# marbl/meryl

Measured on AMD Instinct MI355X. Metric: distinct k-mers counted/sec (whole node), higher is better.
Workload: dtype u64; 1 GPU; meryl count k=21 on synthetic short reads: 66666667 x 150 bp reads per GPU (10.00 Gbp per GPU, 30x of a 333333334 bp genome, 0.5% substitutions, 0.01% N), inputs resident in HBM; k=21, reads_per_gpu=66666667, bases_per_gpu=10066666717, n_distinct=1181289506, parallelism=1 GPU, transport=none (one GPU), n_instances=8648488363, w_prefix=18

## Files before the change

include/meryl_gpu_count.h:

```cpp
#ifndef MERYL_GPU_COUNT_H
#define MERYL_GPU_COUNT_H

#include <stddef.h>
#include <stdint.h>

#ifdef __cplusplus
extern "C" {
#endif

#define MGC_OK            0
#define MGC_EINVAL       -1
#define MGC_ENOMEM       -2
#define MGC_EHIP         -3
#define MGC_ESTATE       -4
#define MGC_EUNSUPPORTED -5
#define MGC_ETIMEOUT     -6
#define MGC_EFORMAT      -7

#define MGC_MODE_CANONICAL 0
#define MGC_MODE_FORWARD   1
#define MGC_MODE_REVERSE   2

#define MGC_NUM_FILES_BITS 6
#define MGC_NUM_FILES      64
// ... 253 lines not shown

int mgc_begin_bam(mgc_session *s);
int mgc_push_bam(mgc_session *s, const void *bam_bytes, size_t len);
int mgc_end_bam(mgc_session *s);
int mgc_push_bam_file(mgc_session *s, const char *path, int threads);
int mgc_dev_bam_decode(const uint8_t *d_piece, uint64_t piece_bytes, const void *d_segments, uint64_t n_segments, uint64_t out_bytes,
                       uint8_t *d_out, void *stream);

int mgc_push_bases_device(mgc_session *s, const uint8_t *d_bases, uint64_t n_bases);

int mgc_staged_bases(mgc_session *s, const uint8_t **d_bases, uint64_t *n_bases);

int mgc_count(mgc_session *s);

int mgc_count_partitioned(mgc_session *s, void *d_keys, const uint64_t *file_counts , void *reserved);

int mgc_count_buckets(mgc_session *s, void *d_keys, uint32_t bucket_bits, const uint64_t *bucket_counts);
int mgc_count_buckets_into(mgc_session *s, void *d_keys, uint32_t bucket_bits, const uint64_t *bucket_counts,
                           void *d_out_keys, uint32_t *d_out_counts, uint64_t capacity, uint64_t *n_distinct,
                           const uint64_t *d_fine_hist );

typedef struct mgc_result_info {
  uint64_t n_bases;
  uint64_t n_instances;
  uint64_t n_distinct;
  uint32_t w_prefix, w_data;
  uint64_t n_prefix;
  uint64_t file_instances[MGC_NUM_FILES];
} mgc_result_info;
int mgc_get_result_info(const mgc_session *s, mgc_result_info *info);

int mgc_copy_result_device(mgc_session *s, void *d_keys_out, uint32_t *d_counts_out);

int mgc_get_result_device(const mgc_session *s, const void **d_unique, const uint32_t **d_counts,
                          const uint64_t **d_block_start, uint32_t *key_words);

int mgc_copy_result(const mgc_session *s, uint64_t *keys_lo, uint64_t *keys_hi, uint32_t *counts,
                    uint64_t *block_start);

typedef int (*mgc_block_cb)(void *ctx, uint64_t prefix, uint64_t n_kmers,
                            const uint64_t *suffix_lo, const uint64_t *suffix_hi,
                            const uint32_t *counts);
int mgc_finish(mgc_session *s, mgc_block_cb cb, void *ctx, int host_threads);

typedef int (*mgc_block_cb2)(void *ctx, uint64_t prefix, uint64_t n_kmers,
                             const uint64_t *suffix_lo, const uint64_t *suffix_hi,
                             const uint32_t *counts, const uint64_t *labels, uint64_t label);
int mgc_finish_labelled(mgc_session *s, mgc_block_cb2 cb, void *ctx, int host_threads);

#define MGC_STAGE_HISTOGRAM 0
#define MGC_STAGE_PARTITION 1
#define MGC_STAGE_SORT      2
#define MGC_STAGE_RLE       3
#define MGC_STAGE_BLOCKS    4
#define MGC_NUM_STAGES      5
typedef struct mgc_profile {
  double   stage_ms[MGC_NUM_STAGES];
  uint32_t stage_launches[MGC_NUM_STAGES];
  double   sort_pass_ms_total;
  uint32_t sort_pass_launches;
  uint64_t sort_pass_keys;
  double   total_ms;
  double   merge_ms;
  uint32_t n_batches;
  uint32_t narrow_digit_widths;
  double   pass_ms[2];
  uint64_t pass_bytes[2];
  uint64_t pass_keys[2];
  uint32_t pass_launches[2];
  double   finish_ms;
  uint64_t finish_bytes, finish_keys;
  uint32_t finish_launches;
  uint32_t wide_msd_files;
  uint32_t stream_files;
  uint32_t k96_files;
  uint32_t k96_widened_files;
  uint32_t hpc_mixed_files;
  uint64_t stream_retries;
  double   probe_ratio;
  double   pack_ms;
  uint64_t hist_bytes;
  uint64_t partition_bytes;
  uint32_t pass_kernel_launches[2];
} mgc_profile;
int mgc_set_profiling(mgc_session *s, int enable);
int mgc_get_profile(const mgc_session *s, mgc_profile *p);

int mgc_dev_synth_reads(uint64_t seed, uint64_t genome_len, uint64_t first_read, uint64_t n_reads,
                        uint32_t read_len, uint32_t sub_rate_ppm, uint32_t n_rate_ppm,
                        uint8_t *d_out, void *stream);
int mgc_dev_synth_reads_ex(uint64_t seed, uint64_t genome_len, uint64_t first_read, uint64_t n_reads,
                           uint32_t read_len, uint32_t sub_rate_ppm, uint32_t n_rate_ppm,
                           uint32_t repeat_ppm, uint32_t repeat_unit, uint32_t repeat_families,
                           uint8_t *d_out, void *stream);

uint32_t mgc_version(void);

#ifdef __cplusplus
}
#endif
#endif
```

meryl_amd/build.py:

```python
import os
import shutil
import subprocess
import sys

HERE = os.path.dirname(os.path.abspath(__file__))
CSRC = os.path.join(HERE, "csrc")
LIB = os.path.join(HERE, "libmeryl_gpu_count.so")
SOURCES = ["mgc_kmer.hip", "mgc_sort.hip", "mgc_scan.hip", "mgc_finish.hip", "mgc_misc.hip", "mgc_parse.hip",
           "mgc_encode.hip", "mgc_decode.hip", "mgc_merge.hip", "mgc_merge_many.hip", "mgc_lookup.hip", "mgc_filter.hip", "mgc_import.hip", "mgc_analyze.hip", "mgc_value_hist.hip", "mgc_positions.hip", "mgc_list.hip", "mgc_bam.hip", "mgc_gzip.hip",
           "mgc_api.cpp", "mgc_textfile.cpp", "mgc_import.cpp", "mgc_analyze.cpp", "mgc_dbfile.cpp", "mgc_positions.cpp", "mgc_count.cpp", "mgc_stream.cpp", "mgc_eval.cpp", "mgc_runs.cpp", "mgc_node.cpp", "meryl_db.cpp", "meryl_seq.cpp"]
HEADERS = ["mgc_device.h", "mgc_common.hpp", "mgc_compact.hpp", "mgc_bases.hpp", "mgc_stream_geom.hpp", "mdb_layout.h", "mdb_statistics.hpp", "mgc_session.hpp", "mgc_devbuf.hpp", "mgc_dbfile.hpp", "mgc_hist_list.hpp", "mgc_clock.hpp", "mgc_chunk_ring.hpp", "mgc_bgzf.hpp", "mgc_bam_walk.hpp", "mgc_gzip_par.hpp", "mgc_runs.hpp", "mgc_lookup_dev.hpp", "mgc_import_dev.hpp", "mgc_analyze_dev.hpp", "mgc_positions_dev.hpp", "mgc_fastx.hpp", "mgc_label.hpp", "mgc_selector.hpp", "mgc_value.hpp", "mgc_route.hpp", "mgc_group_route.hpp", "mgc_group_batch.hpp", "mgc_list.hpp",
           os.path.join("..", "..", "include", "meryl_gpu_count.h"),
           os.path.join("..", "..", "include", "meryl_db.h"), os.path.join("..", "..", "include", "meryl_seq.h"),
           os.path.join("..", "..", "include", "meryl_lookup.h"), os.path.join("..", "..", "include", "meryl_import.h"),
           os.path.join("..", "..", "include", "meryl_import_labelled.h"),
           os.path.join("..", "..", "include", "meryl_analyze.h"), os.path.join("..", "..", "include", "meryl_positions.h"),
           os.path.join("..", "..", "include", "meryl_list.h")]
OBJDIR = os.path.join(HERE, "build")
CFLAGS = ["--offload-arch=gfx950", "-O3", "-std=c++17", "-fPIC", "-pthread", "-Wall", "-Wno-unused-function"]
LFLAGS = ["--offload-arch=gfx950", "-shared", "-fPIC", "-pthread", "-no-hip-rt"]


def hipcc():
    for cand in (os.environ.get("HIPCC"), shutil.which("hipcc"), "/opt/rocm/bin/hipcc"):
        if cand and os.path.exists(cand):
            return cand
    raise RuntimeError("hipcc not found: the native library cannot be built")


def _sources():
    return [f for f in SOURCES if os.path.exists(os.path.join(CSRC, f))]


def _header_mtime():
    deps = [os.path.join(CSRC, f) for f in HEADERS if os.path.exists(os.path.join(CSRC, f))]
    deps.append(os.path.abspath(__file__))
    return max(os.path.getmtime(d) for d in deps)


def _obj(f):
    return os.path.join(OBJDIR, f + ".o")


def _stale_objects(force=False):
    ht = _header_mtime()
    out = []
    for f in _sources():
        o = _obj(f)
        if force or not os.path.exists(o) or os.path.getmtime(o) < max(os.path.getmtime(os.path.join(CSRC, f)), ht):
            out.append(f)
    return out


def _stale():
    if not os.path.exists(LIB):
        return True
    t = os.path.getmtime(LIB)
    if max([_header_mtime()] + [os.path.getmtime(os.path.join(CSRC, f)) for f in _sources()]) <= t:
        return False
    if _stale_objects():
        return True
    return any(os.path.getmtime(_obj(f)) > t for f in _sources())


CLI = os.path.join(HERE, "bin", "meryl")
LOOKUP_CLI = os.path.join(HERE, "bin", "meryl-lookup")
IMPORT_CLI = os.path.join(HERE, "bin", "meryl-import")
ANALYZE_CLI = os.path.join(HERE, "bin", "meryl-analyze")
POSITION_LOOKUP_CLI = os.path.join(HERE, "bin", "position-lookup")


def _build_front_end(source, out, force, verbose, headers=()):
    src = os.path.join(CSRC, source)
    newest = max(os.path.getmtime(os.path.join(CSRC, f)) for f in (source,) + tuple(headers))
    if (not force and os.path.exists(out) and os.path.getmtime(out) >= newest
            and os.path.getmtime(out) >= os.path.getmtime(LIB)):
        return out
    os.makedirs(os.path.dirname(out), exist_ok=True)
    rocm_lib = os.path.join(os.environ.get("ROCM_PATH", "/opt/rocm"), "lib")
    tmp = "%s.tmp%d" % (out, os.getpid())
    cmd = [hipcc(), "-O2", "-std=c++17", "-pthread", src, "-o", tmp, "-L" + HERE, "-lmeryl_gpu_count",
           "-Wl,-rpath,$ORIGIN/..", "-L" + rocm_lib, "-lamdhip64", "-Wl,-rpath," + rocm_lib, "-lz"]
    if verbose:
        print(" ".join(cmd), file=sys.stderr)
    subprocess.check_call(cmd)
    os.replace(tmp, out)
    return out


def build_cli(force=False, verbose=False):
    return _build_front_end("meryl_main.cpp", CLI, force, verbose)


def build_lookup_cli(force=False, verbose=False):
# ... 57 lines not shown
```

meryl_amd/capi.py:

```python
import ctypes
import os

from . import build as _build

MGC_OK, MGC_EINVAL, MGC_ENOMEM, MGC_EHIP, MGC_ESTATE, MGC_EUNSUPPORTED, MGC_ETIMEOUT = 0, -1, -2, -3, -4, -5, -6
MODE_CANONICAL, MODE_FORWARD, MODE_REVERSE = 0, 1, 2
NUM_FILES = 64
NUM_STAGES = 5
STAGE_NAMES = ("histogram", "partition", "sort", "rle", "blocks")

SYMBOLS = (
    "mgc_configure_counting", "mgc_format_configured_line",
    "mgc_dev_partition_workspace_bytes", "mgc_dev_kmer_histogram", "mgc_dev_kmer_partition",
    "mgc_dev_sort_workspace_bytes", "mgc_dev_radix_sort", "mgc_dev_radix_group", "mgc_dev_kmer_histogram_fine",
    "mgc_dev_rle_workspace_bytes", "mgc_dev_rle_count", "mgc_dev_rle_emit", "mgc_dev_block_offsets",
    "mgc_open", "mgc_close", "mgc_last_error", "mgc_push_bases", "mgc_push_bases_device", "mgc_staged_bases", "mgc_reserve_text", "mgc_begin_text", "mgc_push_text", "mgc_end_text", "mgc_push_text_file", "mgc_push_text_file_range", "mgc_text_record_start", "mgc_push_text_bgzf_file", "mgc_is_bgzf_file", "mgc_begin_bam", "mgc_push_bam", "mgc_end_bam", "mgc_push_bam_file", "mgc_dev_bam_decode", "mgc_push_text_gzip_file", "mgc_is_gzip_file", "mgc_dev_gzip_resolve", "mgc_dev_crc32_pieces", "mgc_count", "mgc_count_partitioned", "mgc_count_buckets", "mgc_count_buckets_into", "mgc_copy_result_device",
    "mgc_get_result_info", "mgc_get_result_device", "mgc_copy_result", "mgc_finish", "mgc_finish_labelled",
    "mgc_set_profiling", "mgc_get_profile", "mgc_dev_synth_reads", "mgc_dev_synth_reads_ex", "mgc_version",
    "mgc_dev_merge_workspace_bytes", "mgc_dev_merge_count", "mgc_dev_merge_count_values", "mgc_dev_merge_emit",
    "mgc_dev_merge_many_tile", "mgc_dev_merge_many_workspace_bytes", "mgc_dev_merge_many_count", "mgc_dev_merge_many_emit",
    "mgc_dev_select_workspace_bytes", "mgc_dev_select_count", "mgc_dev_select_emit",
    "mgc_label_default_constant", "mgc_dev_merge_many_emit_labelled", "mgc_dev_select_emit_labelled", "mgc_dev_decode_blocks", "mgc_dev_buffers_live",
    "mgc_select_parse", "mgc_select_check", "mgc_dev_merge_many_count_selected", "mgc_dev_merge_many_emit_selected",
    "mgc_dev_select_count_selected", "mgc_dev_select_emit_selected",
# ... 78 lines not shown
        ("base_mask", ctypes.c_uint8),
        ("reserved", ctypes.c_uint8 * 3),
        ("lhs_index", ctypes.c_int32),
        ("rhs_index", ctypes.c_int32),
        ("lhs_constant", ctypes.c_uint64),
        ("rhs_constant", ctypes.c_uint64),
        ("count_mask", ctypes.c_uint64),
        ("required_mask", ctypes.c_uint32),
        ("reserved2", ctypes.c_uint32),
    ]


class EvalNodeSelected(ctypes.Structure):
    _fields_ = EvalNodeLabelled._fields_ + [
        ("first_term", ctypes.c_uint32),
        ("n_terms", ctypes.c_uint32),
    ]


class EvalNodeAssigned(ctypes.Structure):
    _fields_ = EvalNodeSelected._fields_ + [
        ("value_assign", ctypes.c_int32),
        ("reserved2", ctypes.c_int32),
        ("value_constant", ctypes.c_uint64),
    ]


ASSIGN_OPS = {"none": 0, "set": 1, "first": 2, "selected": 3, "min": 4, "max": 5, "add": 6, "sum": 6, "sub": 7, "dif": 7, "mul": 8, "div": 9,
              "divzero": 10, "mod": 11, "rem": 11, "count": 12}
SEL_VALUE, SEL_LABEL, SEL_BASES, SEL_INPUT = 1, 2, 3, 4
REL_EQ, REL_NEQ, REL_LEQ, REL_GEQ, REL_LT, REL_GT = 1, 2, 3, 4, 5, 6
SELECT_MAX_TERMS = 16
NODE_DATABASE, NODE_MERGE, NODE_VALUE = 0, 1, 2
LABEL_OPS = {"default": 0, "set": 1, "first": 2, "min": 3, "max": 4, "and": 5, "or": 6, "xor": 7, "difference": 8, "lightest": 9,
             "heaviest": 10, "invert": 11, "selected": 12}
EVAL_SLICE_LABELLED_CB = ctypes.CFUNCTYPE(None, ctypes.c_void_p, ctypes.c_uint32, ctypes.POINTER(ctypes.c_uint64), ctypes.POINTER(ctypes.c_uint64),
                                          ctypes.POINTER(ctypes.c_uint32), ctypes.POINTER(ctypes.c_uint64), ctypes.c_uint64)
EVAL_SLICE_CB = ctypes.CFUNCTYPE(None, ctypes.c_void_p, ctypes.c_uint32, ctypes.POINTER(ctypes.c_uint64), ctypes.POINTER(ctypes.c_uint64),
                                 ctypes.POINTER(ctypes.c_uint32), ctypes.c_uint64)


class ResultInfo(ctypes.Structure):
    _fields_ = [
        ("n_bases", ctypes.c_uint64),
        ("n_instances", ctypes.c_uint64),
        ("n_distinct", ctypes.c_uint64),
        ("w_prefix", ctypes.c_uint32),
        ("w_data", ctypes.c_uint32),
        ("n_prefix", ctypes.c_uint64),
        ("file_instances", ctypes.c_uint64 * NUM_FILES),
    ]


class Profile(ctypes.Structure):
    _fields_ = [
        ("stage_ms", ctypes.c_double * NUM_STAGES),
        ("stage_launches", ctypes.c_uint32 * NUM_STAGES),
        ("sort_pass_ms_total", ctypes.c_double),
        ("sort_pass_launches", ctypes.c_uint32),
        ("sort_pass_keys", ctypes.c_uint64),
        ("total_ms", ctypes.c_double),
        ("merge_ms", ctypes.c_double),
        ("n_batches", ctypes.c_uint32),
        ("narrow_digit_widths", ctypes.c_uint32),
        ("pass_ms", ctypes.c_double * 2),
        ("pass_bytes", ctypes.c_uint64 * 2),
        ("pass_keys", ctypes.c_uint64 * 2),
        ("pass_launches", ctypes.c_uint32 * 2),
        ("finish_ms", ctypes.c_double),
        ("finish_bytes", ctypes.c_uint64),
        ("finish_keys", ctypes.c_uint64),
        ("finish_launches", ctypes.c_uint32),
        ("wide_msd_files", ctypes.c_uint32),
        ("stream_files", ctypes.c_uint32),
        ("k96_files", ctypes.c_uint32),
        ("k96_widened_files", ctypes.c_uint32),
        ("hpc_mixed_files", ctypes.c_uint32),
        ("stream_retries", ctypes.c_uint64),
        ("probe_ratio", ctypes.c_double),
        ("pack_ms", ctypes.c_double),
        ("hist_bytes", ctypes.c_uint64),
        ("partition_bytes", ctypes.c_uint64),
        ("pass_kernel_launches", ctypes.c_uint32 * 2),
    ]


class DbInfo(ctypes.Structure):
    _fields_ = [
        ("k", ctypes.c_uint32),
        ("prefix_size", ctypes.c_uint32),
        ("suffix_size", ctypes.c_uint32),
        ("num_files_bits", ctypes.c_uint32),
        ("num_blocks_bits", ctypes.c_uint32),
        ("flags", ctypes.c_uint32),
        ("num_unique", ctypes.c_uint64),
        ("num_distinct", ctypes.c_uint64),
        ("num_total", ctypes.c_uint64),
        ("hist_len", ctypes.c_uint64),
        ("label_size", ctypes.c_uint32),
        ("reserved", ctypes.c_uint32),
    ]


class NodeProfile(ctypes.Structure):
    _fields_ = [
        ("n_ranks", ctypes.c_uint32),
        ("bucket_bits", ctypes.c_uint32),
        ("n_bases", ctypes.c_uint64),
        ("n_instances", ctypes.c_uint64),
        ("n_distinct", ctypes.c_uint64),
        ("data_bytes", ctypes.c_uint64),
        ("partition_s", ctypes.c_double),
        ("exchange_count_s", ctypes.c_double),
        ("close_s", ctypes.c_double),
        ("merge_parts_s", ctypes.c_double),
        ("total_s", ctypes.c_double),
        ("n_batches", ctypes.c_uint32),
        ("n_host_runs", ctypes.c_uint32),
        ("host_run_bytes", ctypes.c_uint64),
        ("merge_runs_s", ctypes.c_double),
        ("peak_hbm_bytes", ctypes.c_uint64),
    ]

    def as_dict(self):
        return {n: getattr(self, n) for n, _ in self._fields_}


class DbWriteProfile(ctypes.Structure):
    _fields_ = [
        ("plan_ms", ctypes.c_double),
        ("encode_ms", ctypes.c_double),
        ("copy_write_s", ctypes.c_double),
        ("total_s", ctypes.c_double),
        ("data_bytes", ctypes.c_uint64),
        ("n_kmers", ctypes.c_uint64),
        ("n_blocks", ctypes.c_uint64),
    ]

    def as_dict(self):
        return {n: getattr(self, n) for n, _ in self._fields_}


class RunsProfile(ctypes.Structure):
    _fields_ = [
        ("n_runs", ctypes.c_uint32), ("n_host_runs", ctypes.c_uint32),
        ("n_entries", ctypes.c_uint64),
        ("device_bytes", ctypes.c_uint64), ("host_bytes", ctypes.c_uint64),
        ("n_merged", ctypes.c_uint64),
        ("n_chunks", ctypes.c_uint32),
        ("spill_s", ctypes.c_double),
        ("upload_s", ctypes.c_double), ("merge_ms", ctypes.c_double), ("deliver_s", ctypes.c_double),
        ("peak_hbm_bytes", ctypes.c_uint64),
    ]

    def as_dict(self):
        return {n: getattr(self, n) for n, _ in self._fields_}


class GzipInfo(ctypes.Structure):
    _fields_ = [(n, ctypes.c_uint64) for n in ("members", "chunks", "confirmed", "discarded", "text_bytes", "symbol_bytes", "cuts")]


class LookupInfo(ctypes.Structure):
    _fields_ = [("k", ctypes.c_uint32), ("key_words", ctypes.c_uint32), ("index_bits", ctypes.c_uint32), ("reserved", ctypes.c_uint32),
                ("n_kmers", ctypes.c_uint64), ("n_kmers_in_db", ctypes.c_uint64), ("device_bytes", ctypes.c_uint64)]

# ... 381 lines not shown
```

meryl_amd/csrc/mgc_api.cpp:

```cpp
#include "../../include/meryl_gpu_count.h"
#include "mgc_device.h"
#include "mgc_session.hpp"
#include "mgc_gzip_par.hpp"
#include "mgc_runs.hpp"
#include "mgc_selector.hpp"
#include "mgc_value.hpp"

#include <algorithm>
#include <cstdio>
#include <cstdlib>
#include <cstring>
#include <string>
#include <thread>
#include <vector>

namespace mgc {
std::string &thread_last_error() {
  thread_local std::string e;
  return e;
}

Switches read_switches() {
  Switches sw;
  auto off = [](const char *n) { const char *e = getenv(n); return e && e[0] == '0'; };
  auto on1 = [](const char *n) { const char *e = getenv(n); return e && e[0] == '1'; };
  auto num = [](const char *n, uint64_t d) { const char *e = getenv(n); return (e && *e) ? strtoull(e, nullptr, 10) : d; };
  sw.fine_hist = !off("MGC_FINE_HIST"); sw.hpc_msd = !off("MGC_HPC_MSD"); sw.hpc_digits = !off("MGC_HPC_DIGITS");
  sw.const_k = !off("MGC_KMER_CONST_K"); sw.packed_bases = !off("MGC_PACKED_BASES"); sw.narrow = !off("MGC_NARROW"); sw.wide_msd = !off("MGC_WIDE_MSD");
  sw.group_pipe = !off("MGC_GROUP_PIPE"); sw.soa5 = !off("MGC_SOA5"); sw.k96 = !off("MGC_K96"); sw.finish = !off("MGC_FINISH");
  sw.nolist = on1("MGC_FINISH_NOLIST");
  sw.finish_trace = getenv("MGC_FINISH_TRACE") != nullptr; sw.group_dbg = getenv("MGC_GROUP_DBG") != nullptr; sw.hash_dbg = getenv("MGC_HASH_DBG") != nullptr;
  { const char *e = getenv("MGC_HASH_MULTI"); sw.hash_multi = (e && *e) ? atoi(e) : -1; }
  { const char *e = getenv("MGC_HASH_STREAM"); sw.hash_stream = (e && *e) ? atoi(e) : -1; }
  sw.min_top = (uint32_t)num("MGC_FINISH_MIN_TOP", 0);
  sw.finish_target = num("MGC_FINISH_TARGET", 0);
  sw.stream_max = num("MGC_STREAM_MAX", (uint64_t)1 << 22);
  sw.bucket_bases = num("MGC_BUCKET_BASES", 0);
  sw.huge_streams = (uint32_t)num("MGC_HUGE_STREAMS", 4);
  sw.huge_slices = !off("MGC_HUGE_SLICES");
  sw.pass_stagger = (uint32_t)num("MGC_PASS_STAGGER", 0);
  sw.group_batch_bytes = num("MGC_GROUP_BATCH_BYTES", sw.group_batch_bytes);
  sw.group_batch_files = (uint32_t)num("MGC_GROUP_BATCH_FILES", 0);
  return sw;
}
}
using mgc::set_err;

namespace {


uint64_t number_of_bits64(uint64_t v) {
  uint64_t b = 0;
  while (v) { b++; v >>= 1; }
  return b;
}

uint64_t expected_simple_size(uint32_t k, uint64_t n_est, uint32_t suffix_len) {
  if (2 * k - 2 * suffix_len > 42) return UINT64_MAX;
  const uint64_t low_bits  = 16;
  const uint64_t n_entries = (uint64_t)1 << (2 * k - 2 * suffix_len);
  const uint64_t exp_max   = (uint64_t)(0.004 * (double)n_est);
  const uint64_t exp_bits  = number_of_bits64(exp_max) + 1;
  const uint64_t extra     = (exp_bits < low_bits) ? 0 : (exp_bits - low_bits);
  return (n_entries * low_bits + n_entries * extra) / 8;
}

void best_prefix_size(const mgc_count_config &c, uint64_t n_est, uint64_t mem_allowed, uint32_t *best,
                      uint64_t *mem_used) {
  const uint32_t k = c.k;
  const uint32_t seg_bits = c.page_size * 8, seg_bytes = c.page_size;
  *best = 0;
  *mem_used = UINT64_MAX;
  for (uint32_t wp = 1; wp < 2 * k - 1; wp++) {
    const uint64_t n_prefix = (uint64_t)1 << wp;
    const uint64_t kpp = n_est / n_prefix + 1;
    const uint64_t kps = seg_bits / (2 * k - wp);
    const uint64_t spp = kpp / kps + 1;
    if (wp + number_of_bits64(spp) + number_of_bits64(seg_bytes) >= 64) break;
    const uint64_t struct_mem = (uint64_t)c.sizeof_count_array * n_prefix + 8 * n_prefix * spp;
    const uint64_t data_min   = n_prefix * seg_bytes;
    const uint64_t total      = struct_mem + n_prefix * spp * seg_bytes;
    if (struct_mem + data_min > mem_allowed) break;
    if ((wp > 9) && (total + (uint64_t)16 * wp * 1024 * 1024 < *mem_used)) {
      *mem_used = total;
      *best = wp;
    }
    if (total > (uint64_t)16 * *mem_used) break;
  }
}

}

extern "C" uint32_t mgc_version(void) { return (0u << 16) | 3u; }

extern "C" int mgc_configure_counting(mgc_count_config *c) {
  if (!c) return MGC_EINVAL;
  if (c->k == 0 || c->k > 64) {
    set_err(nullptr, "ERROR: Kmer size not supplied with modifier k=<kmer-size>.");
    return MGC_EINVAL;
  }
  if (c->mode < 0 || c->mode > 2) return MGC_EINVAL;
  if (c->page_size == 0) c->page_size = 4096;
  if (c->sizeof_count_array == 0) c->sizeof_count_array = 3232;

  c->use_simple = 0; c->w_prefix = 0; c->n_prefix = 0; c->w_data = 0; c->n_batches = 1; c->memory_used = 0;

  const uint64_t mem_simple = expected_simple_size(c->k, c->n_kmers_estimate, c->count_suffix_length);
  uint64_t mem_complex = UINT64_MAX;
  uint32_t best = 0, n_batches = 1;

  if (c->k > 5) {
    for (n_batches = 1; mem_complex > c->memory_allowed; n_batches++) {
      best_prefix_size(*c, c->n_kmers_estimate / n_batches, c->memory_allowed, &best, &mem_complex);
      if (n_batches > (1u << 20)) {
        set_err(nullptr, "configureCounting: no prefix size fits in %lu bytes", (unsigned long)c->memory_allowed);
        return MGC_EINVAL;
      }
    }
    c->w_prefix = best;
    c->n_prefix = (uint64_t)1 << best;
    c->w_data   = 2 * c->k - best;
  }
  if ((mem_simple < mem_complex) && (mem_simple < c->memory_allowed)) {
    c->use_simple = 1; c->memory_used = mem_simple;
  } else {
// ... 469 lines not shown
    if (2 * cfg->k - 2 * sfx_len > 42) {
      set_err(nullptr, "mgc_open: count-suffix forces simple mode, which takes at most 21 free bases (k - suffix length = %u)", cfg->k - sfx_len);
      return nullptr;
    }
    for (uint32_t i = 0; i < sfx_len; i++) {
      const char ch = cfg->count_suffix[i];
      const bool ok = ch == 'A' || ch == 'C' || ch == 'G' || ch == 'T' || ch == 'a' || ch == 'c' || ch == 'g' || ch == 't';
      if (!ok) { set_err(nullptr, "mgc_open: count-suffix '%s' holds something that is not ACGT", cfg->count_suffix); return nullptr; }
      sfx_test = (sfx_test << 2) | (uint64_t)(((unsigned char)ch >> 1) & 3);
    }
    sfx_mask = (sfx_len == 32) ? ~0ull : (((uint64_t)1 << (2 * sfx_len)) - 1);
    eff.use_simple = 1;
  }
  if (!mgc::effective_geometry(&eff)) return nullptr;
  cfg = &eff;
  if (cfg->k == 0 || cfg->k > 64 || cfg->w_prefix < MGC_NUM_FILES_BITS || cfg->w_prefix > 2 * cfg->k ||
      cfg->w_data != 2 * cfg->k - cfg->w_prefix) {
    set_err(nullptr, "mgc_open: config has not been through mgc_configure_counting (k=%u wPrefix=%u wData=%u)",
            cfg->k, cfg->w_prefix, cfg->w_data);
    return nullptr;
  }

  int ndev = 0;
  hipError_t e = hipGetDeviceCount(&ndev);
  if (e != hipSuccess || ndev == 0) {
    set_err(nullptr, "mgc_open: no HIP device (%s)", hipGetErrorString(e));
    return nullptr;
  }
  mgc_session *s = new mgc_session();
  s->cfg = *cfg;
  s->sfx_mask = sfx_mask;
  s->sfx_test = sfx_test;
  s->key_words = (cfg->k > 32) ? 2u : 1u;
  if (device >= 0) {
    e = hipSetDevice(device);
    if (e != hipSuccess) { set_err(nullptr, "hipSetDevice(%d): %s", device, hipGetErrorString(e)); delete s; return nullptr; }
    s->device = device;
  } else {
    (void)hipGetDevice(&s->device);
  }
  e = hipStreamCreateWithFlags(&s->stream, hipStreamNonBlocking);
  if (e == hipSuccess) e = hipStreamCreateWithFlags(&s->st_in, hipStreamNonBlocking);
  if (e != hipSuccess) { set_err(nullptr, "hipStreamCreate: %s", hipGetErrorString(e)); delete s; return nullptr; }
  if (hipStreamCreateWithFlags(&s->stream2, hipStreamNonBlocking) != hipSuccess ||
      hipEventCreateWithFlags(&s->ev_fork, hipEventDisableTiming) != hipSuccess ||
      hipEventCreateWithFlags(&s->ev_join, hipEventDisableTiming) != hipSuccess) {
    set_err(nullptr, "hipStreamCreate / hipEventCreate failed"); mgc_close(s); return nullptr;
  }
  memset(&s->prof, 0, sizeof(s->prof));
  memset(s->file_instances, 0, sizeof(s->file_instances));
  memset(s->total_file_instances, 0, sizeof(s->total_file_instances));
  s->sw = mgc::read_switches();
  return s;
}

extern "C" void mgc_close(mgc_session *s) {
  if (!s) return;
  if (s->worker_active) { s->worker.join(); s->worker_active = false; }
  s->join_prepare();
  (void)hipSetDevice(s->device);
  if (s->st_in) (void)hipStreamSynchronize(s->st_in);
  s->free_result();
  s->free_garbage();
  s->free_arena();
  delete s->runs;
  s->runs = nullptr;
  for (int i = 0; i < 2; i++) {
    if (s->text_pinned[i]) (void)hipHostFree(s->text_pinned[i]);
    if (s->text_ev[i]) (void)hipEventDestroy(s->text_ev[i]);
    if (s->up_ev[i]) (void)hipEventDestroy(s->up_ev[i]);
    if (s->pin[i]) (void)hipHostFree(s->pin[i]);
    if (s->pin_ev[i]) (void)hipEventDestroy(s->pin_ev[i]);
    if (s->bam_seg_pinned[i]) (void)hipHostFree(s->bam_seg_pinned[i]);
    if (s->gz_sym_pinned[i]) (void)hipHostFree(s->gz_sym_pinned[i]);
    if (s->gz_tab_pinned[i]) (void)hipHostFree(s->gz_tab_pinned[i]);
  }
  for (char *&p : s->text_ring) if (p) { (void)hipHostFree(p); p = nullptr; }
  if (s->st_up) { (void)hipStreamSynchronize(s->st_up); (void)hipStreamDestroy(s->st_up); }
  if (s->st_in) (void)hipStreamDestroy(s->st_in);
  if (s->ev_fork) (void)hipEventDestroy(s->ev_fork);
  if (s->h_stats) (void)hipHostFree(s->h_stats);
  if (s->ev_join) (void)hipEventDestroy(s->ev_join);
  if (s->stream2) (void)hipStreamDestroy(s->stream2);
  for (int i = 0; i < mgc_session::HUGE_EXTRA; i++) if (s->stream_h[i]) (void)hipStreamDestroy(s->stream_h[i]);
  if (s->stream) (void)hipStreamDestroy(s->stream);
  delete s;
}

struct HostParseState { uint64_t out_len, file_start_len; uint32_t state, prev_nl, error, pad; };

static int count_staged_batch(mgc_session *s, int which, uint64_t n);

extern "C" int mgc_prepare(mgc_session *s, uint64_t expected_bases) {
  if (!s) return MGC_EINVAL;
  if (s->borrowed || s->counted || s->prep_active || expected_bases == 0) return MGC_OK;
  HIP_TRY(s, hipSetDevice(s->device));
  size_t free_b = 0, total_b = 0;
  if (hipMemGetInfo(&free_b, &total_b) != hipSuccess) return MGC_OK;
  const uint64_t per_base = 2 + 14ull * s->key_words;
  if (s->batch_limit && expected_bases > s->batch_limit) return MGC_OK;
  if ((double)expected_bases * (double)per_base > 0.8 * (double)free_b) return MGC_OK;
  const size_t bytes = sizeof(uint64_t) * s->key_words * expected_bases;
  s->prep_active = true;
  s->prep_thread = std::thread([s, bytes] {
    (void)hipSetDevice(s->device);
    if (s->ensure(mgc_session::B_X, bytes) != hipSuccess) (void)hipGetLastError();
    (void)mgc::warm_kmer(); (void)mgc::warm_scan(); (void)mgc::warm_sort(); (void)mgc::warm_finish(); (void)mgc::warm_encode(); (void)mgc::warm_value_hist();
    (void)hipGetLastError();
  });
  return MGC_OK;
}

extern "C" int mgc_set_batch_bases(mgc_session *s, uint64_t bases_per_batch) {
  if (!s) return MGC_EINVAL;
  s->batch_limit = bases_per_batch;
  return MGC_OK;
}

static inline int stage_id(int which) { return which ? mgc_session::B_STAGE1 : mgc_session::B_STAGE0; }
static inline uint8_t *stage_ptr(mgc_session *s, int which) { return reinterpret_cast<uint8_t *>(s->buf[stage_id(which)].p); }

static int input_setup(mgc_session *s) {
  if (s->borrowed || s->counted) { set_err(&s->err, "input after device input / count"); return MGC_ESTATE; }
  HIP_TRY(s, hipSetDevice(s->device));
  if (s->state_ready) return MGC_OK;
  if (s->batch_limit == 0) {
    size_t free_b = 0, total_b = 0;
    if (hipMemGetInfo(&free_b, &total_b) == hipSuccess && free_b) {
      const uint64_t per_base = 2 + 14ull * s->key_words;
      s->batch_limit = (uint64_t)((double)free_b * 0.80 / (double)per_base);
    }
    if (s->batch_limit < (1u << 20)) s->batch_limit = 1u << 20;
  }
  HIP_TRY(s, s->ensure(mgc_session::B_TEXT_STATE, mgc::text_parse_state_bytes() + 64));
  HIP_TRY(s, s->ensure_preserve(stage_id(s->fill), 1u << 20, 0, s->st_in));
  HIP_TRY(s, mgc::launch_text_file_op(s->buf[mgc_session::B_TEXT_STATE].p, stage_ptr(s, s->fill), 3, s->st_in));
  s->state_ready = true;
  return MGC_OK;
}

static int resolve_length(mgc_session *s, HostParseState *out = nullptr) {
  HostParseState h;
  HIP_TRY(s, hipMemcpyAsync(&h, s->buf[mgc_session::B_TEXT_STATE].p, sizeof(h), hipMemcpyDeviceToHost, s->st_in));
  HIP_TRY(s, hipStreamSynchronize(s->st_in));
  s->fill_len = h.out_len;
  s->len_inexact = false;
  if (out) *out = h;
  return MGC_OK;
}

static int join_worker(mgc_session *s) {
  if (s->worker_active) {
    const double t0 = mgc::now_s();
    s->worker.join();
    s->tr_join += mgc::now_s() - t0;
    s->worker_active = false;
    if (s->worker_rc != MGC_OK) return s->worker_rc;
  }
  return s->worker_rc;
}

static int flush_pinned(mgc_session *s) {
  if (s->pin_len == 0) return MGC_OK;
  if (s->len_inexact) { const int rc = resolve_length(s); if (rc != MGC_OK) return rc; }
  const int c = s->pin_cur;
  HIP_TRY(s, s->ensure_preserve(stage_id(s->fill), s->fill_len + s->pin_len + 4096, s->fill_len, s->st_in));
// ... 767 lines not shown
```

meryl_amd/csrc/mgc_count.cpp:

```cpp
#include "mgc_session.hpp"
#include "mgc_group_batch.hpp"
#include "mgc_group_route.hpp"

#include <algorithm>
#include <vector>

#define TRY(expr) do { const int rc__ = (expr); if (rc__ != MGC_OK) return rc__; } while (0)

namespace {
using S = mgc_session;

struct StageTimer {
  bool on;
  hipStream_t st;
  hipEvent_t ev[MGC_NUM_STAGES][2];
  bool used[MGC_NUM_STAGES];
  StageTimer(bool enable, hipStream_t s) : on(enable), st(s) {
    for (int i = 0; i < MGC_NUM_STAGES; i++) {
      used[i] = false;
      if (on) { (void)hipEventCreate(&ev[i][0]); (void)hipEventCreate(&ev[i][1]); }
    }
  }
  ~StageTimer() {
    if (on) for (int i = 0; i < MGC_NUM_STAGES; i++) { (void)hipEventDestroy(ev[i][0]); (void)hipEventDestroy(ev[i][1]); }
  }
  void begin(int i) { if (on) { (void)hipEventRecord(ev[i][0], st); used[i] = true; } }
  void end(int i)   { if (on) (void)hipEventRecord(ev[i][1], st); }
};

enum class Group : uint8_t {
  NONE,
  SORT,
  NARROW,
  WIDE,
};

struct FilePlan {
  uint64_t size = 0, start = 0;
  uint32_t top = 0;
  uint32_t top_str = 0;
  mgc::SortPlan sp{};
  Group kind = Group::NONE;
  bool hpc = false;
  bool hpc_stream = false;
  bool hpc_cand = false;
  bool hpc_mixed = false;
  bool stream = false;
  bool k96 = false;
  bool msd_ok = true;
  uint32_t tr_a = 0, tr_b = 0;
  uint64_t gbase = 0, sbase = 0, slots = 0;
  size_t nws_off = 0;
  uint32_t *cnt = nullptr;
  uint64_t maxsub = 0, nlarge = 0, nzcount = 0;
  bool fallback = false;
  uint32_t passes = 0; bool narrowed = false, k96_passes = false;
  int batch_lead = -1;
  uint64_t ngf() const { return size ? (uint64_t)1 << top : 0; }
};

uint32_t plan_bucket_bits(const mgc_count_config &c, const mgc::Switches &sw, uint64_t n_bases) {
  const uint64_t per_bucket = sw.bucket_bases ? sw.bucket_bases
                                              : (c.homopoly_compress ? 60000000ull : 180000000ull);
  const uint32_t step = c.homopoly_compress ? 2u : 1u;
  uint32_t bits = MGC_NUM_FILES_BITS;
  while (bits + step <= MGC_MAX_BUCKET_BITS && bits + step <= 2 * c.k && (n_bases >> bits) > per_bucket) bits += step;
  return bits;
}

struct CountPlan {
  const mgc_count_config &c;
  const mgc::Switches &sw;
  mgc_profile &prof;
  uint32_t kw, bucket_bits, nb, rem_bits, fine_bits;
  bool fine = false;
  bool fine_hpc = false;
  uint64_t max_bucket = 0, ng_total = 0, ns_total = 0;
  uint64_t target = 0, cap = 0, starget = 0;
  bool stream_on = false, hpc_ok = false, hpc_stream_ok = false, hpc_mixed_ok = false;
  std::vector<FilePlan> files;

  CountPlan(const mgc_count_config &c_, const mgc::Switches &sw_, mgc_profile &prof_, uint32_t kw_, uint32_t bucket_bits_)
      : c(c_), sw(sw_), prof(prof_), kw(kw_), bucket_bits(bucket_bits_), nb(1u << bucket_bits_), rem_bits(2 * c_.k - bucket_bits_),
        fine_bits(15u - bucket_bits_), files(nb) {}

// ... 120 lines not shown
    }
  }

  int choose_probe() {
    bool any_cand = false;
    for (const FilePlan &x : files) any_cand = any_cand || x.top_str != 0 || x.hpc_cand;
    if (!any_cand) return -1;
    if (sw.hash_stream == 1) {
      for (FilePlan &x : files) if (x.top_str) take_coarser(x);
      return -1;
    }
    int probe = -1;
    uint64_t best = ~0ull;
    for (uint32_t b = 0; b < nb; b++)
      if (files[b].size >= max_bucket / 16 && files[b].size >= 4096 && files[b].size < best) { best = files[b].size; probe = (int)b; }
    return probe;
  }
  void apply_probe(uint32_t probe) {
    for (uint32_t b = 0; b < nb; b++)
      if (b != probe && (files[b].top_str || (files[b].hpc_cand && !files[b].stream))) take_coarser(files[b]);
  }

  uint32_t soa_mask(bool plain_input) const {
    bool soa = sw.soa5 && plain_input && kw == 1 && nb == 64 && fine && rem_bits > 32 && rem_bits <= 40;
    for (const FilePlan &x : files) if (x.size && !(x.kind == Group::NARROW && x.top)) soa = false;
    return soa ? (1u << (rem_bits - 32)) - 1u : 0u;
  }
  bool k96_layout(bool plain_input) {
    if (!(sw.k96 && plain_input && kw == 2 && nb == 64 && fine && rem_bits <= 96 && !c.homopoly_compress)) return false;
    bool any = false;
    for (FilePlan &x : files) if (x.size && x.kind == Group::WIDE && x.top) { x.k96 = true; any = true; prof.k96_files++; }
    return any;
  }
};

struct Count {
  mgc_session *s;
  const mgc::CountInput &in;
  hipStream_t st;
  const mgc_count_config &c;
  const mgc::Switches &sw;
  mgc_profile &prof;
  const uint32_t k, kw, bucket_bits, nb, rem_bits;
  const size_t kbytes;
  CountPlan plan;
  StageTimer tm;
  hipEvent_t ev_all[2] = {nullptr, nullptr};

  const uint8_t *d_bases;
  uint64_t n_bases, N = 0, nd = 0;
  void *part_ws = nullptr, *sort_ws = nullptr, *rle_ws = nullptr;
  uint64_t *d_counts64 = nullptr, *d_starts = nullptr;
  std::vector<uint64_t> h_meta;
  const uint64_t *d_fine = nullptr, *d_fine_hpc = nullptr;
  void *d_packed = nullptr;
  mgc::SortPlan full{};
  bool use_finish;
  unsigned char *X = nullptr, *Y = nullptr;
  size_t sort_ws_bytes = 0;
  uint32_t *d_err = nullptr;
  uint32_t soa_hi_mask = 0;
  static constexpr uint32_t ev_per_file = 2 * 16;
  std::vector<hipEvent_t> pass_ev;
  uint32_t sort_launch_groups = 0;
  size_t y_base_bytes = 0;
  std::vector<unsigned char> h_batch_tables;
  int group_dbg_left = 2;

  int probe = -1;
  uint64_t *d_substart = nullptr, *d_group = nullptr, *d_stats = nullptr, *d_retrycnt = nullptr;
  uint32_t *d_large = nullptr, *d_nz = nullptr;
  const size_t hdr_bytes = mgc::sort_header_bytes();
  unsigned char *d_nws = nullptr, *d_nhdrs = nullptr;
  std::vector<mgc::DBuf> cnt_extra;
  bool fork_huge = false, forked = false, need_join = false;
  static constexpr int NH = 1 + S::HUGE_EXTRA;
  hipStream_t hstream[NH] = {};
  unsigned char *halt[NH] = {};
  void *hws[NH] = {nullptr, nullptr, nullptr, nullptr};
  size_t hws_bytes = 0;
  int n_huge_streams = 1, huge_next = 0;
  std::vector<std::pair<hipEvent_t, hipEvent_t>> fin_ev;
  uint64_t fin_keys = 0, fin_in_bytes = 0; bool fin_narrow = false;

  Count(mgc_session *s_, const mgc::CountInput &in_, uint32_t bucket_bits_)
      : s(s_), in(in_), st(s_->stream), c(s_->cfg), sw(s_->sw), prof(s_->prof), k(c.k), kw(s_->key_words), bucket_bits(bucket_bits_),
        nb(1u << bucket_bits_), rem_bits(2 * c.k - bucket_bits_), kbytes(sizeof(uint64_t) * kw), plan(c, sw, s_->prof, kw, bucket_bits_),
        tm(s_->profiling, s_->stream), d_bases(s_->d_bases), n_bases(s_->n_bases), h_meta(2 * (size_t)nb, 0), use_finish(sw.finish) {}

  void *seg(uint32_t b) const { return X + kbytes * plan.files[b].start; }
  uint32_t low(const FilePlan &x) const { return rem_bits - x.top; }
  const uint32_t *nz_list(const FilePlan &x) const { return (4 * x.nzcount < 3 * x.ngf() && !sw.nolist) ? d_nz + x.gbase : nullptr; }
  bool msd_file(const FilePlan &x) const {
    return d_fine_hpc ? x.kind == Group::WIDE : (x.kind == Group::NARROW || x.kind == Group::WIDE) && x.msd_ok;
  }
  mgc::FinishFile finish_desc(uint32_t b, bool stream, hipStream_t fst, int hsel) const;
  void take_stats(uint32_t b) {
    const uint64_t *h = s->h_stats + 3 * (size_t)b;
    plan.files[b].maxsub = h[0]; plan.files[b].nlarge = h[1]; plan.files[b].nzcount = h[2];
  }

  int run();
  int compress_bases(); int histogram(); int buffers(); int partition(bool soa, bool k96);
  int count_full();
  int count_finish(); int finish_buffers(); int prepare_headers(); int narrow_prepare(int only, int skip);
  int probe_file(); int group_file(uint32_t b); int stats_file(uint32_t b); int group_all();
  mgc::GroupFile group_desc(uint32_t b); bool batch_file(uint32_t b) const; int group_batches();
  int huge_setup(); int huge_sync_all(); int huge_join_all();
  int finish_file(uint32_t b); int oversized_streams(uint32_t b, bool *stream); int widen_back(uint32_t b, bool *unordered);
  int count_file(uint32_t b, bool stream); int fallback_file(uint32_t b, bool unordered);
  int trace_slices(); int retry(); int scan_pack(); int pack_file(uint32_t b); void finish_profile();
  int block_offsets(); void collect_profile();
};

int Count::compress_bases() {
  if (!c.homopoly_compress || !n_bases || in.keys) return MGC_OK;
  HIP_TRY(s, s->ensure(S::B_HPC, n_bases));
  HIP_TRY(s, s->ensure(S::B_HPC_WS, mgc::hpc_workspace_bytes(n_bases)));
  uint8_t *d_hpc = reinterpret_cast<uint8_t *>(s->buf[S::B_HPC].p);
  void *hws_ = s->buf[S::B_HPC_WS].p;
  HIP_TRY(s, mgc::launch_homopoly_compress(d_bases, n_bases, d_hpc, hws_, st));
  uint64_t n_out = 0;
  HIP_TRY(s, hipMemcpyAsync(&n_out, hws_, sizeof(uint64_t), hipMemcpyDeviceToHost, st));
  HIP_TRY(s, hipStreamSynchronize(st));
  d_bases = d_hpc;
  n_bases = n_out;
  return MGC_OK;
}

int Count::histogram() {
  HIP_TRY(s, s->ensure(S::B_PART_WS, mgc::kp_workspace_bytes(bucket_bits)));
  HIP_TRY(s, s->ensure(S::B_META, sizeof(uint64_t) * nb * 3));
  part_ws = s->buf[S::B_PART_WS].p;
  d_counts64 = reinterpret_cast<uint64_t *>(s->buf[S::B_META].p);
  d_starts = d_counts64 + nb;
  std::vector<uint64_t> h_counts(nb);
  const bool wide_msd_on = sw.wide_msd && !c.homopoly_compress;
  if (!in.keys) {
    if (sw.packed_bases && n_bases) {
      const size_t pb = mgc::kp_packed_bytes(n_bases);
      bool room = s->buf[S::B_PACKED].cap >= pb;
      if (!room) {
        size_t free_b = 0, total_b = 0;
        room = hipMemGetInfo(&free_b, &total_b) == hipSuccess &&
               (double)free_b + (double)s->arena_bytes() >= (double)n_bases * (double)(2 + 14ull * kw) + (double)pb;
      }
      if (room) {
        if (s->ensure(S::B_PACKED, pb) == hipSuccess) d_packed = s->buf[S::B_PACKED].p;
        else (void)hipGetLastError();
      }
    }
    tm.begin(MGC_STAGE_HISTOGRAM);
    if (n_bases >= (1u << 22) && ((kw == 1 && 2 * k - bucket_bits <= 41) || wide_msd_on) && mgc::kmer_histogram_fine_ok(k, bucket_bits, s->sfx_mask, sw)) {
      HIP_TRY(s, s->ensure(S::B_FINE, sizeof(uint64_t) << 15));
      uint64_t *fine = reinterpret_cast<uint64_t *>(s->buf[S::B_FINE].p);
      HIP_TRY(s, mgc::launch_kmer_histogram_fine(d_bases, n_bases, k, c.mode, d_counts64, fine, part_ws, st, sw.const_k, 6, d_packed));
      d_fine = fine;
    } else if (c.homopoly_compress && n_bases >= (1u << 22) && (2 * k - bucket_bits) % 2 == 0 && 2 * k - bucket_bits >= 20 &&
               sw.hpc_digits && mgc::kmer_histogram_hpc_ok(k, bucket_bits, s->sfx_mask, sw)) {
      HIP_TRY(s, s->ensure(S::B_FINE, sizeof(uint64_t) * std::max<size_t>((size_t)1 << 15, mgc::kmer_histogram_hpc_entries(bucket_bits))));
      uint64_t *fine = reinterpret_cast<uint64_t *>(s->buf[S::B_FINE].p);
      HIP_TRY(s, mgc::launch_kmer_histogram_hpc(d_bases, n_bases, k, c.mode, bucket_bits, d_counts64, fine, part_ws, st, sw.const_k, d_packed));
      d_fine_hpc = fine;
    } else
    HIP_TRY(s, mgc::launch_kmer_histogram(d_bases, n_bases, k, c.mode, bucket_bits, d_counts64, part_ws, st, s->sfx_mask, s->sfx_test, d_packed));
    tm.end(MGC_STAGE_HISTOGRAM);
    prof.stage_launches[MGC_STAGE_HISTOGRAM] = 1;
    HIP_TRY(s, hipMemcpyAsync(h_counts.data(), d_counts64, sizeof(uint64_t) * nb, hipMemcpyDeviceToHost, st));
    HIP_TRY(s, hipStreamSynchronize(st));
  } else {
    memcpy(h_counts.data(), in.counts, sizeof(uint64_t) * nb);
    uint64_t n_ext = 0;
    for (uint32_t b = 0; b < nb; b++) n_ext += h_counts[b];
    if (in.fine && sw.fine_hist && bucket_bits <= 8 && n_ext >= (1u << 22) && s->sfx_mask == 0 && !c.homopoly_compress &&
        2 * k >= 15 + 2 && ((kw == 1 && 2 * k - bucket_bits <= 41) || wide_msd_on))
      d_fine = in.fine;
  }
  memset(s->file_instances, 0, sizeof(s->file_instances));
  for (uint32_t b = 0; b < nb; b++) {
    plan.files[b].size = h_counts[b];
    plan.files[b].start = h_meta[b] = N;
    N += h_counts[b];
    plan.max_bucket = std::max(plan.max_bucket, h_counts[b]);
    s->file_instances[b >> (bucket_bits - MGC_NUM_FILES_BITS)] += h_counts[b];
  }
  s->n_instances = N;
  plan.fine = d_fine != nullptr;
  plan.fine_hpc = d_fine_hpc != nullptr;
  return MGC_OK;
}

int Count::buffers() {
  mgc::make_sort_plan(0, rem_bits, &full);
  const bool odd = !use_finish && (full.num_passes & 1u) != 0;
// ... 348 lines not shown
  if (*stream && x.maxsub > sw.stream_max && kw == 2) {
    *stream = false;
  } else if (*stream && x.maxsub > sw.stream_max) {
    uint32_t h_fail[3] = {0, 0, 0};
    HIP_TRY(s, hipMemsetAsync(d_err + 4, 0, 12, st));
    HIP_TRY(s, mgc::launch_finish_probe(finish_desc(b, true, st, 0), sw.stream_max, d_err + 4));
    HIP_TRY(s, hipMemcpyAsync(h_fail, d_err + 4, 12, hipMemcpyDeviceToHost, st));
    HIP_TRY(s, hipStreamSynchronize(st));
    *stream = (h_fail[0] == 0);
    if (sw.finish_trace)
      fprintf(stderr, "[finish] bucket %u: largest sub-bucket %llu > %llu, up to %u distinct in one: %s\n", b,
              (unsigned long long)x.maxsub, (unsigned long long)sw.stream_max, h_fail[2],
              *stream ? "streamed through the hash tables" : "too many distinct: stable-sort fallback");
  } else if (sw.finish_trace && x.maxsub > plan.cap) {
    fprintf(stderr, "[finish] bucket %u: largest sub-bucket %llu > %llu: %s\n", b, (unsigned long long)x.maxsub,
            (unsigned long long)plan.cap, *stream ? "streamed through the hash tables" : "stable-sort fallback");
  }
  return MGC_OK;
}

int Count::widen_back(uint32_t b, bool *unordered) {
  FilePlan &x = plan.files[b];
  if (need_join) TRY(huge_sync_all());
  forked = false;
  if (x.k96) {
    const unsigned __int128 fb = (unsigned __int128)b << rem_bits;
    HIP_TRY(s, mgc::launch_widen_k96(seg(b), x.size, (uint64_t)fb, (uint64_t)(fb >> 64), (void *)Y, st));
  } else {
    HIP_TRY(s, mgc::launch_widen_groups(seg(b), d_substart + x.sbase, x.ngf(), (uint64_t)b << rem_bits, low(x), (void *)Y, st, x.tr_a, x.tr_b));
  }
  HIP_TRY(s, hipMemcpyAsync(seg(b), Y, kbytes * x.size, hipMemcpyDeviceToDevice, st));
  if (x.k96) {
    x.k96 = false;
    prof.k96_widened_files++;
    return MGC_OK;
  }
  x.kind = Group::SORT;
  *unordered = x.tr_a != 0;
  if (x.stream) { x.stream = false; *unordered = true; }
  cnt_extra.emplace_back();
  HIP_TRY(s, cnt_extra.back().ensure(sizeof(uint32_t) * x.size));
  x.cnt = reinterpret_cast<uint32_t *>(cnt_extra.back().p);
  return MGC_OK;
}

mgc::FinishFile Count::finish_desc(uint32_t b, bool stream, hipStream_t fst, int hsel) const {
  const FilePlan &x = plan.files[b];
  mgc::FinishFile f;
  f.keys = seg(b); f.alt = halt[hsel];
  f.layout = x.kind == Group::NARROW ? mgc::FinishKeys::NARROW32 : x.k96 ? mgc::FinishKeys::K96 : kw == 2 ? mgc::FinishKeys::WHOLE16 : mgc::FinishKeys::WHOLE8;
  f.starts = d_substart + x.sbase; f.ng = x.ngf(); f.low_bits = low(x); f.tr_a = x.tr_a; f.tr_b = x.tr_b;
  f.n_keys = x.size; f.max_sub = x.maxsub;
  f.cnt_tmp = x.cnt; f.group_distinct = d_group + x.gbase;
  f.large_list = d_large + x.gbase; f.n_large = x.nlarge; f.stream = stream;
  f.nonempty_list = nz_list(x); f.nonempty_count = d_stats + 3 * (size_t)b + 2;
  f.retry_list = x.stream ? d_large + x.gbase + x.nlarge : d_nz + x.gbase; f.retry_count = d_retrycnt + b;
  f.stream_cap = x.stream ? mgc::finish_stream_capacity() : 0;
  f.huge_ws = hws[hsel]; f.huge_ws_bytes = hws_bytes; f.huge_ws_keys = plan.max_bucket; f.d_error = d_err;
  f.st = fst; f.st_huge = hstream[hsel];
  f.hash_multi = sw.hash_multi; f.hash_dbg = sw.hash_dbg;
  return f;
}

int Count::count_file(uint32_t b, bool stream) {
  const FilePlan &x = plan.files[b];
  const bool on_second = fork_huge && (b & 1u);
  if ((stream || on_second) && fork_huge && !forked) {
    HIP_TRY(s, hipEventRecord(s->ev_fork, st));
    for (int i = 0; i < n_huge_streams; i++) HIP_TRY(s, hipStreamWaitEvent(hstream[i], s->ev_fork, 0));
    forked = need_join = true;
  }
  hipStream_t fst = on_second ? s->stream2 : st;
  const int hsel = (stream && x.nlarge > 0 && n_huge_streams > 1) ? (huge_next++ % n_huge_streams) : 0;
  const bool narrow = x.kind == Group::NARROW;
  if (s->profiling) {
    fin_ev.emplace_back(); (void)hipEventCreate(&fin_ev.back().first); (void)hipEventCreate(&fin_ev.back().second);
    (void)hipEventRecord(fin_ev.back().first, fst);
    fin_keys += x.size;
    fin_in_bytes += x.size * (narrow ? 4u : (x.k96 ? 12u : (uint64_t)kbytes));
    fin_narrow = fin_narrow || narrow;
  }
  HIP_TRY(s, mgc::launch_finish_file(finish_desc(b, stream, fst, hsel)));
  if (s->profiling) (void)hipEventRecord(fin_ev.back().second, fst);
  return MGC_OK;
}

int Count::fallback_file(uint32_t b, bool unordered) {
  FilePlan &x = plan.files[b];
  x.fallback = true;
  if (need_join) TRY(huge_sync_all());
  forked = false;
  if (low(x) || unordered) {
    int in_alt = 0;
    HIP_TRY(s, mgc::launch_radix_sort(seg(b), (void *)Y, x.size, kw, full, sort_ws, sort_ws_bytes - 256, d_err, &in_alt, st, nullptr));
    if (in_alt) HIP_TRY(s, hipMemcpyAsync(seg(b), Y, kbytes * x.size, hipMemcpyDeviceToDevice, st));
  }
  uint64_t distinct = 0;
  HIP_TRY(s, mgc::launch_rle_count(seg(b), x.size, kw, rle_ws, st));
  HIP_TRY(s, mgc::rle_read_total(rle_ws, &distinct, st));
  HIP_TRY(s, hipMemsetAsync(d_group + x.gbase, 0, sizeof(uint64_t) * x.slots, st));
  HIP_TRY(s, hipMemcpyAsync(d_group + x.gbase, &distinct, sizeof(uint64_t), hipMemcpyHostToDevice, st));
  HIP_TRY(s, hipStreamSynchronize(st));
  return MGC_OK;
}

int Count::trace_slices() {
  if (!sw.finish_trace || !hws[0]) return MGC_OK;
  HIP_TRY(s, hipStreamSynchronize(st));
  for (int i = 0; i < n_huge_streams; i++) {
    if (!hws[i]) continue;
    mgc::HugeTrace t;
    HIP_TRY(s, mgc::finish_huge_trace(hws[i], plan.max_bucket, &t));
    fprintf(stderr, "[finish] sliced count, stream %d: the last file had %u sub-buckets cut into %u slices; %u of them dense (counted by ranges)\n", i, t.cut, t.slices, t.dense);
  }
  return MGC_OK;
}

int Count::retry() {
  bool any_stream = false;
  for (const FilePlan &x : plan.files) any_stream = any_stream || (x.stream && !x.fallback && x.size);
  if (!any_stream) return MGC_OK;
  std::vector<uint64_t> h_retry(nb, 0);
  HIP_TRY(s, hipMemcpyAsync(h_retry.data(), d_retrycnt, sizeof(uint64_t) * nb, hipMemcpyDeviceToHost, st));
  HIP_TRY(s, hipStreamSynchronize(st));
  for (uint32_t b = 0; b < nb; b++) {
    const FilePlan &x = plan.files[b];
    if (!x.stream || x.fallback || h_retry[b] == 0) continue;
    prof.stream_retries += h_retry[b];
    HIP_TRY(s, mgc::launch_finish_retry(finish_desc(b, true, st, 0), h_retry[b]));
  }
  return MGC_OK;
}

int Count::scan_pack() {
  hipEvent_t ev_pack[2] = {nullptr, nullptr};
  if (s->profiling) { (void)hipEventCreate(&ev_pack[0]); (void)hipEventCreate(&ev_pack[1]); (void)hipEventRecord(ev_pack[0], st); }
  HIP_TRY(s, mgc::launch_finish_scan(d_group, plan.ng_total, s->buf[S::B_GSCAN].p, st));
  HIP_TRY(s, hipMemcpyAsync(&nd, d_group + plan.ng_total, sizeof(uint64_t), hipMemcpyDeviceToHost, st));
  HIP_TRY(s, hipStreamSynchronize(st));
  if (plan.ng_total == 0) nd = 0;
  s->n_distinct = nd;
  if (in.out_keys && in.out_counts && nd <= in.out_cap) {
    s->d_unique = in.out_keys;
    s->d_counts = in.out_counts;
  } else {
    HIP_TRY(s, s->ensure(S::B_UNIQUE, kbytes * nd));
    HIP_TRY(s, s->ensure(S::B_COUNTS, sizeof(uint32_t) * nd));
    s->d_unique = s->buf[S::B_UNIQUE].p;
    s->d_counts = reinterpret_cast<uint32_t *>(s->buf[S::B_COUNTS].p);
  }
  for (uint32_t b = 0; b < nb; b++) TRY(pack_file(b));
  if (s->profiling) (void)hipEventRecord(ev_pack[1], st);
  tm.end(MGC_STAGE_RLE);
  prof.stage_launches[MGC_STAGE_RLE] = 4 * nb;
  if (s->profiling) {
    HIP_TRY(s, hipStreamSynchronize(st));
    { float pms = 0; if (hipEventElapsedTime(&pms, ev_pack[0], ev_pack[1]) == hipSuccess) prof.pack_ms = pms; }
    (void)hipEventDestroy(ev_pack[0]); (void)hipEventDestroy(ev_pack[1]);
    finish_profile();
  }
  return MGC_OK;
}

int Count::pack_file(uint32_t b) {
  const FilePlan &x = plan.files[b];
  if (x.size == 0) return MGC_OK;
  void *sg = seg(b);
  if (x.kind == Group::NARROW) {
    HIP_TRY(s, mgc::launch_compact_groups_narrow(sg, x.cnt, d_substart + x.sbase, d_group + x.gbase, x.ngf(), (uint64_t)b << rem_bits, low(x),
                                                 s->d_unique, s->d_counts, st, x.tr_a, x.tr_b, nz_list(x), x.nzcount));
  } else if (!x.fallback && x.k96) {
    const unsigned __int128 fb = (unsigned __int128)b << rem_bits;
    HIP_TRY(s, mgc::launch_compact_groups_k96(sg, x.cnt, d_substart + x.sbase, d_group + x.gbase, x.ngf(), (uint64_t)fb, (uint64_t)(fb >> 64),
                                              s->d_unique, s->d_counts, st, x.tr_a, x.tr_b, nz_list(x), x.nzcount));
  } else if (!x.fallback) {
    HIP_TRY(s, mgc::launch_compact_groups(sg, kw, x.cnt, d_substart + x.sbase, d_group + x.gbase, x.ngf(), s->d_unique, s->d_counts, st,
                                          x.tr_a, x.tr_b, nz_list(x), x.nzcount));
  } else {
    HIP_TRY(s, mgc::launch_rle_count(sg, x.size, kw, rle_ws, st));
    HIP_TRY(s, mgc::launch_rle_emit(sg, x.size, kw, rle_ws, s->d_unique, s->d_counts, st, d_group + x.gbase));
  }
  return MGC_OK;
}

void Count::finish_profile() {
  for (auto &pe : fin_ev) {
    float ms = 0;
    if (hipEventElapsedTime(&ms, pe.first, pe.second) == hipSuccess) { prof.finish_ms += ms; prof.finish_launches++; }
    (void)hipEventDestroy(pe.first); (void)hipEventDestroy(pe.second);
  }
  prof.finish_keys = fin_keys;
  prof.finish_bytes = fin_in_bytes + nd * (fin_narrow ? 8u : (uint64_t)kbytes + 4u);
}

int Count::count_finish() {
  plan.plan_files();
  probe = plan.choose_probe();
  TRY(finish_buffers());
  soa_hi_mask = plan.soa_mask(!in.keys && s->sfx_mask == 0);
  const bool k96 = plan.k96_layout(!in.keys && s->sfx_mask == 0);
  for (uint32_t b = 0; b < nb; b++) h_meta[nb + b] = plan.files[b].k96 ? 1 : 0;
  TRY(partition(soa_hi_mask != 0, k96));
  uint64_t wide_total = 0;
  for (const FilePlan &x : plan.files) if (x.kind != Group::NARROW) wide_total += x.size;
  HIP_TRY(s, s->ensure(S::B_CNT_TMP, sizeof(uint32_t) * wide_total));
  uint32_t *wide = reinterpret_cast<uint32_t *>(s->buf[S::B_CNT_TMP].p);
  uint64_t at = 0;
  for (uint32_t b = 0; b < nb; b++) {
    FilePlan &x = plan.files[b];
    if (x.kind == Group::NARROW) x.cnt = reinterpret_cast<uint32_t *>(seg(b)) + x.size;
    else { x.cnt = wide + at; at += x.size; }
  }
  tm.begin(MGC_STAGE_SORT);
  TRY(prepare_headers());
  if (s->h_stats_cap < 3 * (size_t)nb) {
    if (s->h_stats) { (void)hipHostFree(s->h_stats); s->h_stats = nullptr; s->h_stats_cap = 0; }
    HIP_TRY(s, hipHostMalloc(reinterpret_cast<void **>(&s->h_stats), sizeof(uint64_t) * 3 * (size_t)nb, hipHostMallocDefault));
    s->h_stats_cap = 3 * (size_t)nb;
  }
  fork_huge = s->stream2 != nullptr;
  hstream[0] = fork_huge ? s->stream2 : st;
  halt[0] = Y;
  hws_bytes = mgc::finish_huge_workspace_bytes(plan.max_bucket);
  if (probe >= 0) TRY(probe_file());
  TRY(group_all());
  for (uint32_t b = 0; b < nb; b++) if ((int)b != probe) TRY(finish_file(b));
  if (need_join) TRY(huge_join_all());
  TRY(trace_slices());
  TRY(retry());
  return scan_pack();
}

int Count::block_offsets() {
  HIP_TRY(s, s->ensure(S::B_BLOCKS, sizeof(uint64_t) * (c.n_prefix + 1)));
  s->d_block_start = reinterpret_cast<uint64_t *>(s->buf[S::B_BLOCKS].p);
  tm.begin(MGC_STAGE_BLOCKS);
  HIP_TRY(s, mgc::launch_block_offsets(s->d_unique, nd, kw, c.w_data, c.n_prefix, s->d_block_start, st));
  tm.end(MGC_STAGE_BLOCKS);
  prof.stage_launches[MGC_STAGE_BLOCKS] = 1;
  uint32_t h_err[3] = {0, 0, 0};
  HIP_TRY(s, hipMemcpyAsync(h_err, d_err, sizeof(h_err), hipMemcpyDeviceToHost, st));
  if (s->profiling) (void)hipEventRecord(ev_all[1], st);
  HIP_TRY(s, hipStreamSynchronize(st));
  if (h_err[0]) { mgc::set_err(&s->err, "radix sort look-back timed out"); return MGC_ETIMEOUT; }
  if (h_err[2]) { mgc::set_err(&s->err, "count stage: the retry table of the distinct-sized count filled up, a sub-bucket was not counted"); return MGC_EHIP; }
  return MGC_OK;
}

void Count::collect_profile() {
  float ms = 0;
  for (int i = 0; i < MGC_NUM_STAGES; i++)
    if (tm.used[i] && hipEventElapsedTime(&ms, tm.ev[i][0], tm.ev[i][1]) == hipSuccess) prof.stage_ms[i] = ms;
  if (hipEventElapsedTime(&ms, ev_all[0], ev_all[1]) == hipSuccess) prof.total_ms = ms;
  prof.stage_launches[MGC_STAGE_SORT] = sort_launch_groups * (full.num_passes + 2);
  for (uint32_t b = 0; b < nb; b++) {
    const FilePlan &x = plan.files[b];
    if (x.size == 0) continue;
    const bool follower = x.batch_lead >= 0 && (uint32_t)x.batch_lead != b;
    for (uint32_t p = 0; p < x.passes; p++) {
      hipEvent_t *pe = &pass_ev[(size_t)b * ev_per_file + 2 * p];
      ms = 0;
      if (!follower && hipEventElapsedTime(&ms, pe[0], pe[1]) != hipSuccess) continue;
      if (!follower) prof.pass_kernel_launches[p ? 1 : 0]++;
      prof.sort_pass_ms_total += ms;
      prof.sort_pass_launches++;
      prof.sort_pass_keys += x.size;
      const int pi = p ? 1 : 0;
      prof.pass_ms[pi] += ms;
      prof.pass_launches[pi]++;
      prof.pass_keys[pi] += x.size;
      if (x.narrowed && !p) prof.narrow_digit_widths |= 1u << (x.tr_a ? x.tr_a : x.sp.pass_bits[0]);
      prof.pass_bytes[pi] += x.size * (x.narrowed ? (p ? 8u : (soa_hi_mask ? 9u : 12u)) : (x.k96_passes ? 24u : 2u * kbytes));
    }
  }
  for (auto &e : pass_ev) (void)hipEventDestroy(e);
  (void)hipEventDestroy(ev_all[0]); (void)hipEventDestroy(ev_all[1]);
  (void)hipGetLastError();
}

int Count::run() {
  TRY(compress_bases());
  if (s->profiling) { (void)hipEventCreate(&ev_all[0]); (void)hipEventCreate(&ev_all[1]); (void)hipEventRecord(ev_all[0], st); }
  TRY(histogram());
  TRY(buffers());
  TRY(use_finish ? count_finish() : count_full());
  TRY(block_offsets());
  if (s->profiling) collect_profile();
  return MGC_OK;
}
}

int mgc::count_device(mgc_session *s, const CountInput &in) {
  s->join_prepare();
  s->free_result();
  HIP_TRY(s, hipSetDevice(s->device));
  const uint32_t bucket_bits = in.keys ? in.bucket_bits : plan_bucket_bits(s->cfg, s->sw, s->n_bases);
  memset(&s->prof, 0, sizeof(s->prof));
  Count count(s, in, bucket_bits);
  return count.run();
}
```

meryl_amd/csrc/mgc_device.h:

```cpp
#pragma once

#include <hip/hip_runtime.h>
#include <stddef.h>
#include <stdint.h>
#include "mgc_label.hpp"
#include "../../include/meryl_gpu_count.h"

namespace mgc {

struct Switches {
  bool fine_hist = true;
  bool hpc_msd = true;
  bool hpc_digits = true;
  bool const_k = true;
  bool packed_bases = true;
  bool narrow = true;
  bool wide_msd = true;
  bool soa5 = true;
  bool group_pipe = true;
  bool k96 = true;
  bool finish = true;
  bool nolist = false;
  bool finish_trace = false;
  bool group_dbg = false;
  uint32_t pass_stagger = 0;
  bool hash_dbg = false;
  int  hash_multi = -1;
  int  hash_stream = -1;
  uint32_t min_top = 0;
  uint64_t finish_target = 0;
  uint64_t stream_max = (uint64_t)1 << 22;
  bool     huge_slices = true;
  uint32_t huge_streams = 4;
  uint64_t bucket_bases = 0;
  uint64_t group_batch_bytes = (uint64_t)1 << 40;
  uint32_t group_batch_files = 0;
};
Switches read_switches();



constexpr int      KP_BLOCK       = 256;
constexpr int      KP_ITEMS       = 16;
constexpr int      KP_TILE        = KP_BLOCK * KP_ITEMS;
constexpr int      KP_MAX_BUCKETS = 1024;

uint32_t kp_grid_size(uint64_t n_bases, uint32_t bucket_bits);
size_t   kp_workspace_bytes(uint32_t bucket_bits);
size_t   kp_packed_bytes(uint64_t n_bases);

bool       kmer_histogram_fine_ok(uint32_t k, uint32_t bucket_bits, uint64_t sfx_mask, const Switches &sw);
bool       kmer_histogram_hpc_ok(uint32_t k, uint32_t bucket_bits, uint64_t sfx_mask, const Switches &sw);
uint32_t   kmer_histogram_hpc_entries(uint32_t bucket_bits);
hipError_t launch_kmer_histogram_hpc(const uint8_t *d_bases, uint64_t n_bases, uint32_t k, int mode, uint32_t bucket_bits,
                                     uint64_t *d_bucket_counts, uint64_t *d_fine_hist, void *d_ws, hipStream_t st, bool const_k = true ,
                                     void *d_packed = nullptr);
hipError_t launch_kmer_histogram_fine(const uint8_t *d_bases, uint64_t n_bases, uint32_t k, int mode, uint64_t *d_bucket_counts,
                                      uint64_t *d_fine_hist, void *d_ws, hipStream_t st, bool const_k = true ,
                                      uint32_t bucket_bits = 6 ,
                                      void *d_packed = nullptr);
bool       kmer_histogram_fine_bits_ok(uint32_t k, uint32_t bucket_bits);
hipError_t launch_kmer_histogram(const uint8_t *d_bases, uint64_t n_bases, uint32_t k, int mode,
                                 uint32_t bucket_bits, uint64_t *d_bucket_counts, void *d_ws, hipStream_t st,
                                 uint64_t sfx_mask = 0, uint64_t sfx_test = 0, void *d_packed = nullptr);
hipError_t launch_kmer_partition(const uint8_t *d_bases, uint64_t n_bases, uint32_t k, int mode,
                                 uint32_t bucket_bits, const uint64_t *d_bucket_starts, void *d_keys,
                                 void *d_ws, hipStream_t st, uint64_t sfx_mask = 0, uint64_t sfx_test = 0,
                                 const uint64_t *d_soa_counts = nullptr ,
                                 bool const_k = true , void *d_packed = nullptr);

struct SortPlan {
  uint32_t radix_bits;
  uint32_t block;
  uint32_t kpt;
  uint32_t tile;
  uint32_t mode;
  uint32_t hpc;
  uint32_t num_passes;
  uint32_t pass_shift[16];
  uint32_t pass_bits[16];
};

void   make_sort_plan(uint32_t begin_bit, uint32_t end_bit, SortPlan *plan);
void   make_hpc_group_plan(uint32_t low_bit, uint32_t passes, SortPlan *plan);
void   make_hpc_mixed_plan(uint32_t low_bit, SortPlan *plan);
size_t sort_workspace_bytes(uint64_t n);

hipError_t launch_radix_sort(void *d_keys, void *d_alt, uint64_t n, uint32_t key_words, const SortPlan &plan,
                             void *d_ws, size_t ws_bytes, uint32_t *d_error, int *result_in_alt,
                             hipStream_t st, hipEvent_t *pass_events );
size_t     sort_header_bytes();
enum class GroupKeys : uint32_t {
  U64,
  SOA5,
  K128,
  K96,
};
struct GroupFile {
  void *keys = nullptr, *alt = nullptr;
  uint64_t n = 0;
  const SortPlan *plan = nullptr;
  GroupKeys layout = GroupKeys::U64;
  uint32_t soa_hi_mask = 0;
  uint32_t *d_error = nullptr;
  uint64_t *d_sub_starts = nullptr;
  hipStream_t st = nullptr;
  hipEvent_t *pass_events = nullptr;
  void *prepared = nullptr, *scratch = nullptr;
  void *ws = nullptr; size_t ws_bytes = 0;
  bool pipe = false;
  uint32_t stagger = 0;
  bool dbg = false;
  uint32_t tr_a = 0, tr_b = 0;
};
bool       sort_plan_narrows(const SortPlan &plan, uint64_t n, uint32_t key_words, bool on = true );
size_t     narrow_scratch_bytes(uint64_t n);
hipError_t launch_narrow_prepare(const uint64_t *d_fine, uint32_t nb, const unsigned char *bits_a, const unsigned char *on, void *d_hdrs,
                                 hipStream_t st);
hipError_t launch_group_narrow(GroupFile &f);
struct GroupBatch {
  GroupFile *files = nullptr; uint32_t nfiles = 0;
  void *d_table = nullptr, *h_table = nullptr;
  uint32_t *d_ctl = nullptr;
  uint32_t *d_error = nullptr;
  hipStream_t st = nullptr;
  hipEvent_t *pass_events = nullptr;
};
size_t     group_batch_table_bytes(uint32_t nfiles);
hipError_t launch_group_narrow_batch(GroupBatch &b);
bool       sort_plan_wide_msd(const SortPlan &plan, uint64_t n, bool on = true );
hipError_t launch_hpc_prepare(const uint64_t *d_fine_hpc, uint32_t bucket_bits, const uint64_t on[4], void *d_hdrs, hipStream_t st);
size_t     wide_scratch_bytes(uint64_t n, uint32_t key_words);
hipError_t launch_group_wide(GroupFile &f);

size_t     rle_workspace_bytes(uint64_t n);
hipError_t launch_rle_count(const void *d_sorted, uint64_t n, uint32_t key_words, void *d_ws, hipStream_t st);
hipError_t rle_read_total(const void *d_ws, uint64_t *n_distinct, hipStream_t st);
hipError_t launch_rle_emit(const void *d_sorted, uint64_t n, uint32_t key_words, void *d_ws, void *d_unique,
                           uint32_t *d_counts, hipStream_t st, const uint64_t *d_out_base = nullptr);

uint64_t   finish_capacity_for(uint32_t key_words);
uint64_t   finish_target_for(uint32_t key_words, const Switches &sw);
bool       finish_stream_ok(uint32_t key_words, uint32_t low_bits, bool narrow = true);
uint64_t   finish_stream_capacity();
uint64_t   finish_stream_target(const Switches &sw);
uint64_t   finish_stream_distinct();
hipError_t launch_subbucket_bounds(const void *d_keys, uint64_t n, uint32_t key_words, uint32_t low, uint32_t top_bits,
                                   uint64_t *d_starts , uint64_t *d_max ,
                                   uint32_t *d_large_list ,
                                   uint64_t *d_large_count ,
                                   uint32_t *d_nonempty_list , uint64_t *d_nonempty_count ,
                                   hipStream_t st);
hipError_t launch_subbucket_max(const uint64_t *d_starts, uint32_t key_words, uint32_t low, uint32_t top_bits, uint64_t *d_max,
                                uint32_t *d_large_list, uint64_t *d_large_count, uint32_t *d_nonempty_list, uint64_t *d_nonempty_count,
                                hipStream_t st, uint64_t small_cap = 0 );
bool       finish_uses_hash(uint32_t key_words, uint32_t low_bits);
enum class FinishKeys : uint32_t {
  WHOLE8,
  NARROW32,
  K96,
  WHOLE16,
};
struct FinishFile {
  void *keys = nullptr;
  void *alt = nullptr;
  FinishKeys layout = FinishKeys::WHOLE8;
  const uint64_t *starts = nullptr;
  uint64_t ng = 0;
  uint32_t low_bits = 0;
  uint32_t tr_a = 0, tr_b = 0;
  uint64_t n_keys = 0;
  uint64_t max_sub = 0;
  uint32_t *cnt_tmp = nullptr;
  uint64_t *group_distinct = nullptr;
  const uint32_t *large_list = nullptr;
  uint64_t n_large = 0;
  bool stream = false;
  const uint32_t *nonempty_list = nullptr;
  const uint64_t *nonempty_count = nullptr;
  uint32_t *retry_list = nullptr;
  uint64_t *retry_count = nullptr;
  uint64_t stream_cap = 0;
  void *huge_ws = nullptr; size_t huge_ws_bytes = 0; uint64_t huge_ws_keys = 0;
  uint32_t *d_error = nullptr;
  hipStream_t st = nullptr;
  hipStream_t st_huge = nullptr;
  int  hash_multi = -1;
  bool hash_dbg = false;
};
hipError_t launch_finish_probe(const FinishFile &f, uint64_t stream_max , uint32_t *d_file_fail);
hipError_t launch_finish_file(const FinishFile &f);
hipError_t launch_finish_retry(const FinishFile &f, uint64_t n_retry);
size_t     finish_huge_workspace_bytes(uint64_t n_keys);
struct HugeTrace { uint32_t cut, slices, dense; };
hipError_t finish_huge_trace(const void *d_ws, uint64_t ws_keys, HugeTrace *out);
size_t     finish_scan_scratch_bytes(uint64_t ng_total);
hipError_t launch_finish_scan(uint64_t *d_group , uint64_t ng_total, void *d_scratch, hipStream_t st);
hipError_t launch_compact_groups(const void *d_keys, uint32_t key_words, const uint32_t *d_cnt_tmp, const uint64_t *d_starts,
                                 const uint64_t *d_offs, uint64_t ng, void *d_out_keys, uint32_t *d_out_counts, hipStream_t st,
                                 uint32_t tr_a = 0, uint32_t tr_b = 0 ,
                                 const uint32_t *d_nonempty_list = nullptr, uint64_t n_nonempty = 0 );
hipError_t launch_compact_groups_narrow(const void *d_keys32, const uint32_t *d_cnt_tmp, const uint64_t *d_starts, const uint64_t *d_offs,
                                        uint64_t ng, uint64_t base, uint32_t low_bits, void *d_out_keys, uint32_t *d_out_counts, hipStream_t st,
                                        uint32_t tr_a, uint32_t tr_b, const uint32_t *d_nonempty_list = nullptr, uint64_t n_nonempty = 0);
hipError_t launch_compact_groups_k96(const void *d_keys96, const uint32_t *d_cnt_tmp, const uint64_t *d_starts, const uint64_t *d_offs,
                                     uint64_t ng, uint64_t base_lo, uint64_t base_hi, void *d_out_keys, uint32_t *d_out_counts, hipStream_t st,
                                     uint32_t tr_a, uint32_t tr_b, const uint32_t *d_nonempty_list = nullptr, uint64_t n_nonempty = 0);
hipError_t launch_widen_k96(const void *d_keys96, uint64_t n, uint64_t base_lo, uint64_t base_hi, void *d_out128, hipStream_t st);
hipError_t launch_widen_groups(const void *d_keys32, const uint64_t *d_starts, uint64_t ng, uint64_t base, uint32_t low_bits, void *d_out64,
                               hipStream_t st, uint32_t tr_a, uint32_t tr_b);
hipError_t launch_store_u64(uint64_t *d_dst, const uint64_t *d_src, hipStream_t st);
hipError_t launch_sum_u64(const uint64_t *d_in, uint64_t n, uint64_t *d_out, hipStream_t st);

hipError_t launch_block_offsets(const void *d_unique, uint64_t n_distinct, uint32_t key_words, uint32_t w_data,
                                uint64_t n_prefix, uint64_t *d_block_start, hipStream_t st);

hipError_t launch_block_offsets_range(const void *d_keys, uint64_t n, uint32_t key_words, uint32_t w_data, uint64_t prefix_begin,
                                      uint64_t n_blocks, uint64_t n_prefix_total, uint64_t *d_rel_start, hipStream_t st);
hipError_t launch_encode_sizes(const void *d_keys, uint32_t key_words, const uint64_t *d_bs, uint64_t n_blocks, uint32_t suffix_size,
                               uint32_t label_size, uint64_t *d_blk_bytes, uint64_t *d_blk_vbase, uint32_t *d_blk_bb, hipStream_t st);
hipError_t launch_encode_chunk(const void *d_keys, const uint32_t *d_counts, uint32_t key_words, const uint64_t *d_bs,
                               const uint64_t *d_blk_pos, const uint64_t *d_blk_vbase, const uint32_t *d_blk_bb,
                               uint64_t b0, uint64_t b1, uint64_t n_kmers_chunk, uint64_t prefix_of_block0,
                               uint32_t suffix_size, uint32_t label_size, uint64_t label, void *d_img, hipStream_t st,
                               const uint64_t *d_labels = nullptr );

hipError_t launch_decode_blocks(const void *d_file, const void *d_blocks, uint64_t n_blocks, uint32_t suffix_size, uint32_t label_size,
                                uint32_t key_words, void *d_keys, uint32_t *d_counts, uint32_t *d_err, hipStream_t st,
                                uint64_t *d_labels = nullptr );

size_t     merge_workspace_bytes(uint64_t na, uint64_t nb);
hipError_t launch_merge_count(const void *dA, uint64_t na, const void *dB, uint64_t nb, uint32_t key_words, int op, void *d_ws,
                              hipStream_t st, const uint32_t *cA = nullptr, const uint32_t *cB = nullptr);
hipError_t merge_read_total(const void *d_ws, uint64_t *n_out, hipStream_t st);
hipError_t launch_merge_emit(const void *dA, const uint32_t *cA, uint64_t na, const void *dB, const uint32_t *cB, uint64_t nb,
                             uint32_t key_words, int op, void *d_ws, void *d_out_keys, uint32_t *d_out_counts, hipStream_t st);
struct PassRule {
  int       lop = 0;
  uint64_t  lc = 0;
  bool      select = false;
  const ::mgc_select_term *terms = nullptr;
  uint32_t  n_terms = 0, k = 0;
  int       vop = 0;
  uint64_t  vc = 0;
  int       fop = -1;
  uint64_t  fc = 0;
  uint64_t *out_labs = nullptr;
};
struct MergeManyInputs { const void *const *keys; const uint32_t *const *vals; const uint64_t *const *labs; const uint64_t *n; uint32_t count, key_words; };
uint32_t   merge_many_tile(uint32_t key_words);
size_t     merge_many_workspace_bytes(const uint64_t *n, uint32_t n_inputs, uint32_t key_words);
hipError_t launch_merge_many(bool emit, const MergeManyInputs &in, int op, const PassRule &rule, void *d_ws, void *d_out_keys,
                             uint32_t *d_out_vals, hipStream_t st);
struct SelectInput { const void *keys; const uint32_t *vals; const uint32_t *flags; const uint64_t *labs; uint64_t n; uint32_t key_words; };
size_t     select_workspace_bytes(uint64_t n);
hipError_t launch_select(bool emit, const SelectInput &in, int fop, uint64_t constant, const PassRule &rule, void *d_ws, void *d_out_keys,
                         uint32_t *d_out_vals, hipStream_t st);
hipError_t launch_fill_u32(uint32_t *d, uint64_t n, uint32_t v, hipStream_t st);
hipError_t launch_last_breaker(const uint8_t *d_bases, uint64_t n, uint64_t *d_out, hipStream_t st);

size_t     hpc_workspace_bytes(uint64_t n);
hipError_t launch_homopoly_compress(const uint8_t *d_in, uint64_t n, uint8_t *d_out, void *d_ws, hipStream_t st);

size_t     text_parse_state_bytes();
size_t     text_parse_workspace_bytes(uint64_t n);
hipError_t launch_text_parse(const uint8_t *d_text, uint64_t n, int fastq, void *d_state, void *d_ws, uint8_t *d_out, hipStream_t st);
hipError_t launch_bam_decode(const uint8_t *d_piece, uint64_t piece_bytes, const void *d_segments, uint64_t n_segments, uint64_t out_total,
                             uint8_t *d_out, hipStream_t st);
hipError_t launch_gzip_resolve(uint8_t *d_text, uint64_t text_bytes, const uint16_t *d_symbols, uint64_t n_symbols, const uint8_t *d_window_in,
                               uint32_t window_valid, uint8_t *d_window_out, uint32_t *d_error, hipStream_t st);
hipError_t launch_gzip_crc32(const uint8_t *d_text, const uint64_t *d_begin, const uint32_t *d_len, uint64_t n_pieces, uint32_t *d_crc, hipStream_t st);
hipError_t launch_text_file_op(void *d_state, uint8_t *d_out, int what, hipStream_t st);
hipError_t launch_text_set_len(void *d_state, uint64_t new_len, int rebase_file, hipStream_t st);

hipError_t launch_synth_reads(uint64_t seed, uint64_t genome_len, uint64_t first_read, uint64_t n_reads,
                              uint32_t read_len, uint32_t sub_rate_ppm, uint32_t n_rate_ppm,
                              uint32_t repeat_ppm, uint32_t repeat_unit, uint32_t repeat_families,
                              uint8_t *d_out, hipStream_t st);

hipError_t warm_kmer(); hipError_t warm_sort(); hipError_t warm_finish(); hipError_t warm_encode(); hipError_t warm_scan(); hipError_t warm_value_hist();
}
```

meryl_amd/csrc/mgc_finish.hip:

```cpp
#include "mgc_common.hpp"
#include "mgc_stream_geom.hpp"

#include <algorithm>
#include <type_traits>
#include <vector>

namespace mgc {


constexpr int RL_BLOCK = 256;
constexpr u64 RL_INF   = ~0ull;
template <typename K> struct RlTile { static constexpr int KPT = 16; };
template <> struct RlTile<K128>     { static constexpr int KPT = 8;  };

struct RleWs {
  u64 *total, *tile_offs, *tile_next, *scratch;
  u64  num_tiles;
};
static inline RleWs rle_ws(void *d_ws, uint64_t n, uint32_t key_words) {
  const uint64_t tile = (uint64_t)RL_BLOCK * (key_words == 2 ? RlTile<K128>::KPT : RlTile<u64>::KPT);
  RleWs w;
  w.num_tiles = (n + tile - 1) / tile;
  w.total     = reinterpret_cast<u64 *>(d_ws);
  w.tile_offs = w.total + 8;
// ... 1983 lines not shown
      if (!chain_sent) __hip_atomic_store(hs.chain + (u64)cq * HUGE_RANGES + rr, total | (1ull << 63), __ATOMIC_RELAXED, __HIP_MEMORY_SCOPE_AGENT);
      if (rr == HUGE_RANGES - 1) { hs.gig_dist[cq] = (u32)total; group_distinct[tr_index(g, tr_a, tr_b)] = total; }
    }
    return;
  }
  if (!in_place) {
    __syncthreads();
    for (u64 i = tid; i < out; i += BLOCK) gk[i] = alt[a + i];
  }
  if (tid == 0) group_distinct[tr_index(g, tr_a, tr_b)] = out;
}

template <int BLOCK, int CAP, int SLOTS, bool WIDE, typename KT = K128, int MODE = 0>
__global__ __launch_bounds__(BLOCK)
void hash_count128_huge_kernel(KT *__restrict__ keys, const u64 *__restrict__ starts, const u32 *__restrict__ list, u64 ng,
                               u64 huge_min, u32 low_bits, u32 *__restrict__ cnt_tmp, u64 *__restrict__ group_distinct,
                               KT *__restrict__ alt, u32 tr_a = 0, u32 tr_b = 0, u64 huge_max = 0, HugeSliced hs = HugeSliced()) {
  if constexpr (MODE == 0 || MODE == 2) {
    hash_count128_huge_body<BLOCK, CAP, SLOTS, WIDE, KT, MODE>(blockIdx.x, keys, starts, list, ng, huge_min, low_bits, cnt_tmp, group_distinct, alt, tr_a, tr_b, huge_max, hs);
  } else {
    __shared__ u32 s_ticket;
    for (;;) {
      __syncthreads();
      if (threadIdx.x == 0) s_ticket = atomicAdd(&hs.counters[MODE == 1 ? 3 : 2], 1u);
      __syncthreads();
      const u32 item = s_ticket;
      if (item >= (MODE == 1 ? hs.counters[1] : hs.counters[0] * HUGE_RANGES)) return;
      hash_count128_huge_body<BLOCK, CAP, SLOTS, WIDE, KT, MODE>(item, keys, starts, list, ng, huge_min, low_bits, cnt_tmp, group_distinct, alt, tr_a, tr_b, huge_max, hs);
    }
  }
}

template <typename S, int BLOCK, int CAP, int SLOTS, typename KT = u64>
__global__ __launch_bounds__(BLOCK)
void hash_probe_kernel(const KT *__restrict__ keys, const u64 *__restrict__ starts, const u32 *__restrict__ list,
                       u64 huge_min, u32 low_bits, u32 *__restrict__ file_fail) {
  constexpr int KPT = CAP / BLOCK;
  const S EMPTY = ~(S)0;
  __shared__ S   tk[SLOTS];
  __shared__ u32 s_st[2];
  const u32 tid = threadIdx.x;
  const u64 g = list[blockIdx.x];
  const u64 a = starts[g], n64 = starts[g + 1] - a;
  if (n64 <= huge_min) return;
  const u64 low_mask = (low_bits >= 64) ? ~0ull : ((1ull << low_bits) - 1ull);
  for (u32 i = tid; i < (u32)SLOTS; i += BLOCK) tk[i] = EMPTY;
  if (tid < 2) s_st[tid] = 0u;
  __syncthreads();
  constexpr u32 smask = SLOTS - 1, sshift = 32 - __builtin_ctz((unsigned)SLOTS);
  for (u64 base = 0; base < n64; base += (u64)CAP) {
    S   kk[KPT];
    u32 hh[KPT], pending = 0;
#pragma unroll
    for (int j = 0; j < KPT; j++) {
      const u64 idx = base + (u64)j * BLOCK + tid;
      kk[j] = (idx < n64) ? (S)((u64)keys[a + idx] & low_mask) : (S)0;
      hh[j] = (u32)(((u64)kk[j] * 0x9E3779B97F4A7C15ull) >> 32) >> sshift;
      if (idx < n64) pending |= 1u << j;
    }
    while (pending && !__hip_atomic_load(&s_st[1], __ATOMIC_RELAXED, __HIP_MEMORY_SCOPE_WORKGROUP)) {
#pragma unroll
      for (int j = 0; j < KPT; j++) {
        if ((pending >> j) & 1u) {
          const S old = atomicCAS(&tk[hh[j]], EMPTY, kk[j]);
          if (old == EMPTY || old == kk[j]) {
            pending &= ~(1u << j);
            if (old == EMPTY && atomicAdd(&s_st[0], 1u) >= (u32)CAP) s_st[1] = 1u;
          }
          else hh[j] = (hh[j] + 1) & smask;
        }
      }
    }
    if (__hip_atomic_load(&s_st[1], __ATOMIC_RELAXED, __HIP_MEMORY_SCOPE_WORKGROUP)) break;
  }
  __syncthreads();
  if (tid == 0 && s_st[1]) atomicExch(file_fail, 1u);
  if (tid == 0) atomicMax(file_fail + 2, s_st[0]);
}

template <typename K>
__global__ __launch_bounds__(256)
void compact_groups_kernel(const K *__restrict__ keys, const u32 *__restrict__ cnt_tmp, const u64 *__restrict__ starts,
                           const u64 *__restrict__ offs, u64 ng, K *__restrict__ out_keys, u32 *__restrict__ out_counts, u32 tr_a, u32 tr_b,
                           const u32 *__restrict__ nz, u64 n_nz ) {
  u64 g = (u64)blockIdx.x * 4 + wave_id();
  if (nz) { if (g >= n_nz) return; g = nz[g]; }
  else if (g >= ng) return;
  const u64 gt = tr_index(g, tr_a, tr_b);
  const u64 dst = offs[gt], d = offs[gt + 1] - dst, src = starts[g];
  for (u64 i = lane_id(); i < d; i += 64) {
    out_keys[dst + i]   = keys[src + i];
    out_counts[dst + i] = cnt_tmp[src + i];
  }
}

__global__ __launch_bounds__(256)
void compact_groups_k96_kernel(const K96 *__restrict__ keys, const u32 *__restrict__ cnt_tmp, const u64 *__restrict__ starts,
                               const u64 *__restrict__ offs, u64 ng, u64 base_lo, u64 base_hi, K128 *__restrict__ out_keys,
                               u32 *__restrict__ out_counts, u32 tr_a, u32 tr_b, const u32 *__restrict__ nz, u64 n_nz) {
  u64 g = (u64)blockIdx.x * 4 + wave_id();
  if (nz) { if (g >= n_nz) return; g = nz[g]; }
  else if (g >= ng) return;
  const u64 gt = tr_index(g, tr_a, tr_b);
  const u64 dst = offs[gt], d = offs[gt + 1] - dst, src = starts[g];
  for (u64 i = lane_id(); i < d; i += 64) {
    const K96 q = keys[src + i];
    K128 o; o.lo = KeyOps<K96>::low64(q) | base_lo; o.hi = (u64)q.w[2] | base_hi;
    out_keys[dst + i]   = o;
    out_counts[dst + i] = cnt_tmp[src + i];
  }
}
__global__ __launch_bounds__(256)
void widen_k96_kernel(const K96 *__restrict__ in, u64 n, u64 base_lo, u64 base_hi, K128 *__restrict__ out) {
  for (u64 i = (u64)blockIdx.x * 256 + threadIdx.x; i < n; i += (u64)gridDim.x * 256) {
    const K96 q = in[i];
    K128 o; o.lo = KeyOps<K96>::low64(q) | base_lo; o.hi = (u64)q.w[2] | base_hi;
    out[i] = o;
  }
}

__global__ __launch_bounds__(256)
void compact_groups_narrow_kernel(const u32 *__restrict__ keys32, const u32 *__restrict__ cnt_tmp, const u64 *__restrict__ starts,
                                  const u64 *__restrict__ offs, u64 ng, u64 base, u32 low_bits, u64 *__restrict__ out_keys,
                                  u32 *__restrict__ out_counts, u32 tr_a, u32 tr_b, const u32 *__restrict__ nz, u64 n_nz) {
  u64 g = (u64)blockIdx.x * 4 + wave_id();
  if (nz) { if (g >= n_nz) return; g = nz[g]; }
  else if (g >= ng) return;
  const u64 gt = tr_index(g, tr_a, tr_b);
  const u64 dst = offs[gt], d = offs[gt + 1] - dst, src = starts[g], pre = base | (gt << low_bits);
  for (u64 i = lane_id(); i < d; i += 64) {
    out_keys[dst + i]   = pre | (u64)keys32[src + i];
    out_counts[dst + i] = cnt_tmp[src + i];
  }
}

__global__ __launch_bounds__(256)
void widen_groups_kernel(const u32 *__restrict__ keys32, const u64 *__restrict__ starts, u64 ng, u64 base, u32 low_bits,
                         u64 *__restrict__ out, u32 tr_a, u32 tr_b) {
  const u64 g = (u64)blockIdx.x * 4 + wave_id();
  if (g >= ng) return;
  const u64 a = starts[g], e = starts[g + 1], pre = base | (tr_index(g, tr_a, tr_b) << low_bits);
  const u32 low_mask = (low_bits >= 32) ? ~0u : ((1u << low_bits) - 1u);
  for (u64 i = a + lane_id(); i < e; i += 64) out[i] = pre | (u64)(keys32[i] & low_mask);
}

__global__ void store_u64_kernel(u64 *__restrict__ dst, const u64 *__restrict__ src) { *dst = *src; }

constexpr u64 FIN_CAP_SMALL = 256 * 16, FIN_CAP_LARGE = 1024 * 8;
constexpr int HUGE_CAP32 = 4096, HUGE_SLOTS32 = 8192;
constexpr int HUGE_CAP64 = 2048, HUGE_SLOTS64 = 4096;
constexpr int HUGE_CAP128 = 2048, HUGE_SLOTS128 = 4096;
constexpr size_t HUGE_LDS32 = (size_t)(4 + 4) * HUGE_SLOTS32 + (size_t)(4 + 4) * HUGE_CAP32 + 16 * 4;
constexpr size_t HUGE_LDS64 = (size_t)(8 + 4) * HUGE_SLOTS64 + (size_t)(8 + 4) * HUGE_CAP64 + 16 * 8;
constexpr size_t HUGE_LDS128 = (size_t)(8 + 4) * HUGE_SLOTS128 + (size_t)8 * (HUGE_CAP128 + 16) + (size_t)4 * HUGE_CAP128;
constexpr size_t HUGE_LDS128_WIDE = (size_t)(8 + 8 + 4) * HUGE_SLOTS128 + (size_t)(8 + 8) * (HUGE_CAP128 + 16) + (size_t)4 * HUGE_CAP128;
constexpr u64 FIN_CAP_HASH  = 1536;
constexpr u64 FIN_CAP_STREAM = 4094;
constexpr int FIN_STREAM_KPC = 6, FIN_STREAM_SLOTS = 2048, FIN_STREAM_DCAP = 1280, FIN_STREAM_RETRY_SLOTS = 8192, FIN_STREAM_RETRY_DCAP = 4096;
constexpr int FIN_STREAM64_DCAP = 1024;

constexpr u64 FIN_CAP_HASH128 = 1536;

bool finish_uses_hash(uint32_t key_words, uint32_t low_bits) {
  if (key_words == 2) return low_bits <= 122;
  return key_words == 1 && low_bits <= 58;
}
static uint64_t finish_small_capacity(uint32_t key_words, uint32_t low_bits);

hipError_t launch_subbucket_bounds(const void *d_keys, uint64_t n, uint32_t key_words, uint32_t low, uint32_t top_bits,
                                   uint64_t *d_starts, uint64_t *d_max, uint32_t *d_list, uint64_t *d_list_count,
                                   uint32_t *d_nz, uint64_t *d_nz_count, hipStream_t st) {
  const uint64_t ng = (uint64_t)1 << top_bits;
  const uint32_t tmask = (uint32_t)(ng - 1);
  const dim3 grid((uint32_t)((ng + 1 + 255) / 256));
  if (key_words == 2)
    hipLaunchKernelGGL(subbucket_bounds_kernel<K128>, grid, dim3(256), 0, st, reinterpret_cast<const K128 *>(d_keys),
                       (u64)n, low, tmask, (u64)ng, reinterpret_cast<u64 *>(d_starts));
  else
    hipLaunchKernelGGL(subbucket_bounds_kernel<u64>, grid, dim3(256), 0, st, reinterpret_cast<const u64 *>(d_keys),
                       (u64)n, low, tmask, (u64)ng, reinterpret_cast<u64 *>(d_starts));
  MGC_CHECK(hipGetLastError());
  return launch_subbucket_max(d_starts, key_words, low, top_bits, d_max, d_list, d_list_count, d_nz, d_nz_count, st);
}

hipError_t launch_subbucket_max(const uint64_t *d_starts, uint32_t key_words, uint32_t low, uint32_t top_bits, uint64_t *d_max,
                                uint32_t *d_list, uint64_t *d_list_count, uint32_t *d_nz, uint64_t *d_nz_count, hipStream_t st,
                                uint64_t small_cap) {
  const uint64_t ng = (uint64_t)1 << top_bits;
  hipLaunchKernelGGL(subbucket_max_kernel, dim3((uint32_t)((ng + 255) / 256)), dim3(256), 0, st,
                     reinterpret_cast<const u64 *>(d_starts), (u64)ng, reinterpret_cast<u64 *>(d_max),
                     (u64)(small_cap ? small_cap : finish_small_capacity(key_words, low)), d_list, reinterpret_cast<u64 *>(d_list_count),
                     d_nz, reinterpret_cast<u64 *>(d_nz_count));
  return hipGetLastError();
}

static uint32_t finish_key_words(FinishKeys layout) { return (layout == FinishKeys::K96 || layout == FinishKeys::WHOLE16) ? 2u : 1u; }
static const u64 *fin_starts(const FinishFile &f) { return reinterpret_cast<const u64 *>(f.starts); }
static u64 *fin_distinct(const FinishFile &f) { return reinterpret_cast<u64 *>(f.group_distinct); }
static uint32_t fin_grid(uint64_t items, uint32_t max_wgs) { return items < max_wgs ? (uint32_t)items : max_wgs; }

template <typename F> static hipError_t with_bools(F &&fn) { return fn(); }
template <typename F, typename... B> static hipError_t with_bools(F &&fn, bool b, B... rest) {
  return b ? with_bools([&](auto... c) { return fn(std::true_type(), c...); }, rest...)
           : with_bools([&](auto... c) { return fn(std::false_type(), c...); }, rest...);
}

template <typename K, int BLOCK, int KPT>
// ... 278 lines not shown
    MGC_CHECK((wide ? launch_countw<K128, true>(f, small) : launch_countw<K128, false>(f, small)));
    break;
  case FinishPath::K128_SORT:
    MGC_CHECK((launch_lds_sort<K128, 256, 8>(f, f.ng, 0, 2048)));
    break;
  case FinishPath::NARROW_STREAM: {
    u64 *dbg = hash_dbg_buffer(f.hash_dbg);
    if (list)     MGC_CHECK((launch_stream<u32, FIN_STREAM_SLOTS, FIN_STREAM_DCAP, true, false>(f, f.ng, 256u * 16u, f.nonempty_list, f.nonempty_count, f.retry_list, f.retry_count)));
    else if (dbg) MGC_CHECK((launch_stream<u32, FIN_STREAM_SLOTS, FIN_STREAM_DCAP, false, true>(f, f.ng, 256u * 16u, nullptr, nullptr, f.retry_list, f.retry_count, dbg)));
    else          MGC_CHECK((launch_stream<u32, FIN_STREAM_SLOTS, FIN_STREAM_DCAP, false, false>(f, f.ng, 256u * 16u, nullptr, nullptr, f.retry_list, f.retry_count)));
    break;
  }
  case FinishPath::NARROW_MULTI1:
    MGC_CHECK((launch_multi<1, false>(f, hash_dbg_buffer(f.hash_dbg))));
    break;
  case FinishPath::NARROW_MULTI2:
  case FinishPath::NARROW_MULTI4: {
    u64 *dbg = hash_dbg_buffer(f.hash_dbg);
    if (path == FinishPath::NARROW_MULTI4) MGC_CHECK((launch_multi<4, false>(f, dbg)));
    else if (dbg)                            MGC_CHECK((launch_multi<2, true>(f, dbg)));
    else                                     MGC_CHECK((launch_multi<2, false>(f, dbg)));
    MGC_CHECK(launch_hash_count<true>(f, 256u * 7u, f.retry_list, f.retry_count, nullptr));
    break;
  }
  case FinishPath::NARROW_HASH:
    MGC_CHECK(launch_hash_count<true>(f, 256u * 14u, f.nonempty_list, f.nonempty_count, hash_dbg_buffer(f.hash_dbg)));
    break;
  case FinishPath::U64_STREAM:
    if (list) MGC_CHECK((launch_stream<u64, FIN_STREAM_SLOTS, FIN_STREAM64_DCAP, true, false>(f, f.ng, 256u * 10u, f.nonempty_list, f.nonempty_count, f.retry_list, f.retry_count)));
    else      MGC_CHECK((launch_stream<u64, FIN_STREAM_SLOTS, FIN_STREAM64_DCAP, false, false>(f, f.ng, 256u * 10u, nullptr, nullptr, f.retry_list, f.retry_count)));
    break;
  case FinishPath::U64_CLAIMED:
    MGC_CHECK((launch_countw<u64, false>(f, small)));
    break;
  case FinishPath::U64_PACKED:
    MGC_CHECK(launch_hash_count<false>(f, 256u * 14u, f.nonempty_list, f.nonempty_count, hash_dbg_buffer(f.hash_dbg)));
    break;
  case FinishPath::U64_SORT:
    MGC_CHECK((launch_lds_sort<u64, 256, 16>(f, f.ng, 0, FIN_CAP_SMALL)));
    break;
  }
  return launch_oversized(f);
}

hipError_t launch_finish_retry(const FinishFile &f, uint64_t n_retry) {
  const bool narrow = f.layout == FinishKeys::NARROW32;
  if (n_retry == 0) return hipSuccess;
  if (!finish_stream_ok(1, f.low_bits, narrow) || f.stream_cap == 0 || f.stream_cap > FIN_CAP_STREAM) return hipErrorInvalidValue;
  if (!narrow) {
    if (!f.alt) return hipErrorInvalidValue;
    return f.low_bits < 32 ? launch_huge_mode<Huge8<u32, u64>, 0>(f, f.retry_list, (uint32_t)n_retry, 0, 0, HugeSliced(), f.st)
                           : launch_huge_mode<Huge8<u64, u64>, 0>(f, f.retry_list, (uint32_t)n_retry, 0, 0, HugeSliced(), f.st);
  }
  static_assert(FIN_STREAM_RETRY_DCAP >= (int)FIN_CAP_STREAM, "the retry table holds every suffix of a sub-bucket");
  static_assert(FIN_STREAM_RETRY_SLOTS >= 2 * (int)FIN_CAP_STREAM, "... and stays at most half full: every probe ends");
  return launch_stream<u32, FIN_STREAM_RETRY_SLOTS, FIN_STREAM_RETRY_DCAP, true, false, true>(f, n_retry, 256u * 2u, f.retry_list, f.retry_count, nullptr, nullptr);
}

bool     finish_stream_ok(uint32_t key_words, uint32_t low_bits, bool narrow) { return key_words == 1 && low_bits >= 8 && low_bits <= (narrow ? 20u : 52u); }
uint64_t finish_stream_capacity() { return FIN_CAP_STREAM; }
uint64_t finish_stream_distinct() { return FIN_STREAM_DCAP; }
uint64_t finish_stream_target(const Switches &sw) {
  if (sw.finish_target) return sw.finish_target;
  return (FIN_CAP_HASH * 3) / 2;
}

static uint64_t finish_small_capacity(uint32_t key_words, uint32_t low_bits) {
  if (key_words == 2) return finish_uses_hash(key_words, low_bits) ? FIN_CAP_HASH128 : 2048;
  return finish_uses_hash(key_words, low_bits) ? FIN_CAP_HASH : FIN_CAP_SMALL;
}

uint64_t finish_capacity_for(uint32_t key_words) { return key_words == 2 ? 8192 : FIN_CAP_LARGE; }
uint64_t finish_target_for(uint32_t key_words, const Switches &sw) {
  if (sw.finish_target) return sw.finish_target;
  return key_words == 2 ? (FIN_CAP_HASH128 * 3) / 4 : (FIN_CAP_HASH * 3) / 4;
}

size_t finish_scan_scratch_bytes(uint64_t ng_total) { return scan_scratch_elems(ng_total + 1) * sizeof(uint64_t); }
hipError_t launch_finish_scan(uint64_t *d_group, uint64_t ng_total, void *d_scratch, hipStream_t st) {
  return scan_u64_exclusive(reinterpret_cast<u64 *>(d_group), ng_total, reinterpret_cast<u64 *>(d_scratch),
                            reinterpret_cast<u64 *>(d_group) + ng_total, st);
}

hipError_t launch_compact_groups(const void *d_keys, uint32_t key_words, const uint32_t *d_cnt_tmp, const uint64_t *d_starts,
                                 const uint64_t *d_offs, uint64_t ng, void *d_out_keys, uint32_t *d_out_counts, hipStream_t st,
                                 uint32_t tr_a, uint32_t tr_b, const uint32_t *d_nz, uint64_t n_nz) {
  const dim3 grid((uint32_t)(((d_nz ? n_nz : ng) + 3) / 4));
  if (d_nz && n_nz == 0) return hipSuccess;
  if (key_words == 2)
    hipLaunchKernelGGL(compact_groups_kernel<K128>, grid, dim3(256), 0, st, reinterpret_cast<const K128 *>(d_keys), d_cnt_tmp,
                       reinterpret_cast<const u64 *>(d_starts), reinterpret_cast<const u64 *>(d_offs), (u64)ng,
                       reinterpret_cast<K128 *>(d_out_keys), d_out_counts, tr_a, tr_b, d_nz, (u64)n_nz);
  else
    hipLaunchKernelGGL(compact_groups_kernel<u64>, grid, dim3(256), 0, st, reinterpret_cast<const u64 *>(d_keys), d_cnt_tmp,
                       reinterpret_cast<const u64 *>(d_starts), reinterpret_cast<const u64 *>(d_offs), (u64)ng,
                       reinterpret_cast<u64 *>(d_out_keys), d_out_counts, tr_a, tr_b, d_nz, (u64)n_nz);
  return hipGetLastError();
}

hipError_t launch_compact_groups_narrow(const void *d_keys32, const uint32_t *d_cnt_tmp, const uint64_t *d_starts, const uint64_t *d_offs,
                                        uint64_t ng, uint64_t base, uint32_t low_bits, void *d_out_keys, uint32_t *d_out_counts, hipStream_t st,
                                        uint32_t tr_a, uint32_t tr_b, const uint32_t *d_nz, uint64_t n_nz) {
  if (d_nz && n_nz == 0) return hipSuccess;
  hipLaunchKernelGGL(compact_groups_narrow_kernel, dim3((uint32_t)(((d_nz ? n_nz : ng) + 3) / 4)), dim3(256), 0, st, reinterpret_cast<const u32 *>(d_keys32),
                     d_cnt_tmp, reinterpret_cast<const u64 *>(d_starts), reinterpret_cast<const u64 *>(d_offs), (u64)ng, (u64)base, low_bits,
                     reinterpret_cast<u64 *>(d_out_keys), d_out_counts, tr_a, tr_b, d_nz, (u64)n_nz);
  return hipGetLastError();
}

hipError_t launch_compact_groups_k96(const void *d_keys96, const uint32_t *d_cnt_tmp, const uint64_t *d_starts, const uint64_t *d_offs,
                                     uint64_t ng, uint64_t base_lo, uint64_t base_hi, void *d_out_keys, uint32_t *d_out_counts, hipStream_t st,
                                     uint32_t tr_a, uint32_t tr_b, const uint32_t *d_nz, uint64_t n_nz) {
  if (d_nz && n_nz == 0) return hipSuccess;
  hipLaunchKernelGGL(compact_groups_k96_kernel, dim3((uint32_t)(((d_nz ? n_nz : ng) + 3) / 4)), dim3(256), 0, st, reinterpret_cast<const K96 *>(d_keys96),
                     d_cnt_tmp, reinterpret_cast<const u64 *>(d_starts), reinterpret_cast<const u64 *>(d_offs), (u64)ng, (u64)base_lo, (u64)base_hi,
                     reinterpret_cast<K128 *>(d_out_keys), d_out_counts, tr_a, tr_b, d_nz, (u64)n_nz);
  return hipGetLastError();
}

hipError_t launch_widen_k96(const void *d_keys96, uint64_t n, uint64_t base_lo, uint64_t base_hi, void *d_out128, hipStream_t st) {
  if (n == 0) return hipSuccess;
  const uint64_t g = (n + 255) / 256;
  hipLaunchKernelGGL(widen_k96_kernel, dim3((uint32_t)(g < 256u * 32u ? g : 256u * 32u)), dim3(256), 0, st, reinterpret_cast<const K96 *>(d_keys96), (u64)n,
                     (u64)base_lo, (u64)base_hi, reinterpret_cast<K128 *>(d_out128));
  return hipGetLastError();
}

hipError_t launch_widen_groups(const void *d_keys32, const uint64_t *d_starts, uint64_t ng, uint64_t base, uint32_t low_bits, void *d_out64,
                               hipStream_t st, uint32_t tr_a, uint32_t tr_b) {
  hipLaunchKernelGGL(widen_groups_kernel, dim3((uint32_t)((ng + 3) / 4)), dim3(256), 0, st, reinterpret_cast<const u32 *>(d_keys32),
                     reinterpret_cast<const u64 *>(d_starts), (u64)ng, (u64)base, low_bits, reinterpret_cast<u64 *>(d_out64), tr_a, tr_b);
  return hipGetLastError();
}

__global__ __launch_bounds__(256)
void sum_u64_kernel(const u64 *__restrict__ in, u64 n, u64 *__restrict__ out) {
  u64 v = 0;
  for (u64 i = (u64)blockIdx.x * blockDim.x + threadIdx.x; i < n; i += (u64)gridDim.x * blockDim.x) v += in[i];
#pragma unroll
  for (int d = 32; d >= 1; d >>= 1) v += __shfl_down(v, d);
  if (lane_id() == 0 && v) atomicAdd((unsigned long long *)out, v);
}
hipError_t launch_sum_u64(const uint64_t *d_in, uint64_t n, uint64_t *d_out, hipStream_t st) {
  MGC_CHECK(hipMemsetAsync(d_out, 0, sizeof(uint64_t), st));
  if (n == 0) return hipSuccess;
  const uint64_t blocks = (n + 1023) / 1024;
  hipLaunchKernelGGL(sum_u64_kernel, dim3((uint32_t)(blocks < 256 ? blocks : 256)), dim3(256), 0, st, reinterpret_cast<const u64 *>(d_in),
                     (u64)n, reinterpret_cast<u64 *>(d_out));
  return hipGetLastError();
}

hipError_t launch_store_u64(uint64_t *d_dst, const uint64_t *d_src, hipStream_t st) {
  hipLaunchKernelGGL(store_u64_kernel, dim3(1), dim3(1), 0, st, reinterpret_cast<u64 *>(d_dst), reinterpret_cast<const u64 *>(d_src));
  return hipGetLastError();
}

template <typename K>
__global__ void block_offsets_kernel(const K *__restrict__ keys, u64 nd, u32 w_data, u64 n_prefix,
                                     u64 *__restrict__ block_start) {
  const u64 p = (u64)blockIdx.x * blockDim.x + threadIdx.x;
  if (p > n_prefix) return;
  if (p == n_prefix) { block_start[p] = nd; return; }
  const K target = KeyOps<K>::prefix_floor(p, w_data);
  u64 lo = 0, hi = nd;
  while (lo < hi) {
    const u64 mid = lo + ((hi - lo) >> 1);
    if (KeyOps<K>::lt(keys[mid], target)) lo = mid + 1; else hi = mid;
  }
  block_start[p] = lo;
}

hipError_t launch_block_offsets(const void *d_unique, uint64_t n_distinct, uint32_t key_words, uint32_t w_data,
                                uint64_t n_prefix, uint64_t *d_block_start, hipStream_t st) {
  const uint64_t threads = n_prefix + 1;
  const dim3 grid((uint32_t)((threads + 255) / 256));
  if (key_words == 2)
    hipLaunchKernelGGL(block_offsets_kernel<K128>, grid, dim3(256), 0, st, reinterpret_cast<const K128 *>(d_unique),
                       (u64)n_distinct, w_data, (u64)n_prefix, reinterpret_cast<u64 *>(d_block_start));
  else
    hipLaunchKernelGGL(block_offsets_kernel<u64>, grid, dim3(256), 0, st, reinterpret_cast<const u64 *>(d_unique),
                       (u64)n_distinct, w_data, (u64)n_prefix, reinterpret_cast<u64 *>(d_block_start));
  return hipGetLastError();
}


hipError_t warm_finish() { hipFuncAttributes a; return hipFuncGetAttributes(&a, reinterpret_cast<const void *>(&store_u64_kernel)); }

}
```

meryl_amd/csrc/mgc_session.hpp:

```cpp
#pragma once

#include "../../include/meryl_gpu_count.h"
#include "mgc_bam_walk.hpp"
#include "mgc_clock.hpp"
#include "mgc_devbuf.hpp"
#include "mgc_device.h"

#include <cstdarg>
#include <cstdio>
#include <cstring>
#include <mutex>
#include <string>
#include <thread>
#include <vector>

namespace mgc {
std::string &thread_last_error();
bool effective_geometry(mgc_count_config *c);

inline void set_err(std::string *dst, const char *fmt, ...) {
  char buf[512];
  va_list ap;
  va_start(ap, fmt);
  vsnprintf(buf, sizeof(buf), fmt, ap);
  va_end(ap);
  if (dst) {
    static std::mutex mu;
    std::lock_guard<std::mutex> g(mu);
    *dst = buf;
  }
  thread_last_error() = buf;
}
}

#define HIP_TRY(s, expr)                                                                         \
  do {                                                                                           \
    hipError_t e__ = (expr);                                                                     \
    if (e__ != hipSuccess) {                                                                     \
      mgc::set_err((s) ? &(s)->err : nullptr, "%s:%d: %s -> %s", __FILE__, __LINE__, #expr,      \
                   hipGetErrorString(e__));                                                      \
      return (e__ == hipErrorOutOfMemory) ? MGC_ENOMEM : MGC_EHIP;                               \
    }                                                                                            \
  } while (0)

struct mgc_session {
  mgc_count_config cfg;
  int              device = -1;
  hipStream_t      stream = nullptr;
  uint64_t         sfx_mask = 0, sfx_test = 0;
  mgc::Switches    sw;
  static constexpr int HUGE_EXTRA = 3;
  hipStream_t      stream_h[HUGE_EXTRA] = {nullptr, nullptr, nullptr};
  hipStream_t      stream2 = nullptr;
  hipEvent_t       ev_fork = nullptr, ev_join = nullptr;
  uint64_t        *h_stats = nullptr;
  size_t           h_stats_cap = 0;
  std::string      err;

  const uint8_t    *d_bases = nullptr;
  uint64_t          n_bases = 0;
  bool              borrowed = false;

  bool      counted = false;
  uint64_t  n_instances = 0, n_distinct = 0;
  uint64_t  file_instances[MGC_NUM_FILES];
  void     *d_unique = nullptr;
  uint32_t *d_counts = nullptr;
  uint64_t *d_block_start = nullptr;
  uint32_t  key_words = 1;

  struct Buf { void *p = nullptr; size_t cap = 0; };
  enum { B_PART_WS, B_META, B_X, B_Y, B_SORT_WS, B_RLE_WS, B_UNIQUE, B_COUNTS, B_BLOCKS, B_HPC, B_HPC_WS,
         B_SUBSTART, B_GROUPS, B_GSCAN, B_CNT_TMP, B_LARGE, B_NONEMPTY, B_STAGE0, B_STAGE1, B_TEXT_IN0, B_TEXT_IN1, B_TEXT_WS,
         B_TEXT_STATE, B_RK, B_RC, B_R2K, B_R2C, B_MERGE_WS, B_SORT_HDRS, B_FINE, B_NARROW_WS, B_Y2, B_Y3, B_Y4, B_HWS0, B_HWS1, B_HWS2, B_HWS3,
         B_PACKED ,
         B_GROUP_BATCH ,
         B_BAM_SEG0, B_BAM_SEG1 ,
         B_GZ_SYM0, B_GZ_SYM1 , B_GZ_TAB0, B_GZ_TAB1 , B_GZ_WIN , B_NUM };
  Buf buf[B_NUM];
  size_t arena_bytes() const { size_t t = 0; for (const auto &b : buf) t += b.cap; return t; }
  double tr_alloc = 0;
  uint64_t tr_alloc_bytes = 0;
  hipError_t ensure(int which, size_t bytes) {
    Buf &b = buf[which];
    if (bytes < 256) bytes = 256;
    if (b.cap >= bytes) return hipSuccess;
    const double t0 = mgc::now_s();
    if (b.p) { (void)hipFree(b.p); b.p = nullptr; b.cap = 0; }
    hipError_t e = hipMalloc(&b.p, bytes);
    if (e == hipSuccess) b.cap = bytes;
    tr_alloc += mgc::now_s() - t0;
    tr_alloc_bytes += bytes;
    return e;
  }
  void free_arena() { for (auto &b : buf) { if (b.p) (void)hipFree(b.p); b.p = nullptr; b.cap = 0; } }
  std::vector<void *> garbage;
  hipError_t ensure_preserve(int which, size_t bytes, size_t keep, hipStream_t on) {
    Buf &b = buf[which];
    if (b.cap >= bytes) return hipSuccess;
    struct Tm { double *acc; double t0; Tm(double *a) : acc(a), t0(mgc::now_s()) {} ~Tm() { *acc += mgc::now_s() - t0; } } tm_(&tr_grow);
    size_t want = b.cap * 4;
    const size_t full = batch_limit ? (size_t)batch_limit + 4 * PIN_CHUNK : 0;
    if (full && want > full && full >= bytes) want = full;
    if (want < bytes) want = bytes;
    void *np = nullptr;
    hipError_t e = hipMalloc(&np, want);
    if (e != hipSuccess && want > bytes) { want = bytes; e = hipMalloc(&np, want); }
    if (e != hipSuccess) return e;
    if (b.p && keep) e = hipMemcpyAsync(np, b.p, keep, hipMemcpyDeviceToDevice, on);
    if (e == hipSuccess) e = hipStreamSynchronize(on);
    if (b.p) garbage.push_back(b.p);
    b.p = np; b.cap = want;
    return e;
  }
  void free_garbage() { for (void *p : garbage) (void)hipFree(p); garbage.clear(); }

  static constexpr size_t TEXT_CHUNK = 32u << 20;
  static constexpr size_t PIN_CHUNK  = 32u << 20;
  hipStream_t st_in = nullptr;
  bool        state_ready = false;
  int         fill = 0;
  uint64_t    fill_len = 0;
  bool        len_inexact = false;
  bool        input_seen = false;
  bool        text_open = false, text_cut_in_file = false;
  int         text_format = 0;
  char       *text_pinned[2] = {nullptr, nullptr};
  hipEvent_t  text_ev[2] = {nullptr, nullptr};
  hipStream_t st_up = nullptr;
  hipEvent_t  up_ev[2] = {nullptr, nullptr};
  bool        text_ev_used[2] = {false, false};
  uint32_t    text_next = 0;
  static constexpr int TEXT_RING_MAX = 64;
  char       *text_ring[TEXT_RING_MAX] = {nullptr};
  static constexpr int TEXT_BAM = 3;
  mgc::BamWalker bam_walker;
  std::vector<mgc::BamSegment> bam_segs;
  mgc::BamSegment *bam_seg_pinned[2] = {nullptr, nullptr};
  size_t      bam_seg_cap[2] = {0, 0};
  double      tr_bam_walk = 0;
  struct GzCrcPiece { uint32_t len; int32_t end; };
  struct GzEnd { uint32_t crc, isize; uint64_t comp_off; };
  int         gz_win = 0;
  char       *gz_sym_pinned[2] = {nullptr, nullptr};
  size_t      gz_sym_cap[2] = {0, 0};
  char       *gz_tab_pinned[2] = {nullptr, nullptr};
  size_t      gz_tab_cap[2] = {0, 0};
  std::vector<GzCrcPiece> gz_pending[2];
  std::vector<GzEnd> gz_ends[2];
  uint32_t    gz_crc = 0;
  uint64_t    gz_member_len = 0, gz_members = 0;
  std::string gz_verdict;
  uint64_t    gz_piece_off[2] = {0, 0};
  double      tr_gz_copy = 0, tr_gz_collect = 0, tr_gz_wait = 0;
  char       *pin[2] = {nullptr, nullptr};
  size_t      pin_len = 0;
  int         pin_cur = 0;
  hipEvent_t  pin_ev[2] = {nullptr, nullptr};
  bool        pin_used[2] = {false, false};

  uint64_t    batch_limit = 0;
// ... 56 lines not shown
```

Before: 12.47 billion distinct k-mers/s.

## Overlap per-file packing with remaining finish kernels on a second stream

Adds an early-packing path: after each file's finish kernel, a separate stream runs a gated prefix-scan over that file's group counts and compacts the previous file into the output arrays, so packing overlaps the count/finish of later files instead of running serially at the end. Output buffers are presized from the probe file's distinct/instance ratio plus a margin, and a device-side gate state defers files that would overflow. If the estimate is exceeded, the remaining files fall back to the late scan and pack. This adds events, an extra state buffer and the risk of re-packing everything when the buffers have to move.

```diff
diff --git a/include/meryl_gpu_count.h b/include/meryl_gpu_count.h
--- a/include/meryl_gpu_count.h
+++ b/include/meryl_gpu_count.h
@@ -359,6 +359,9 @@
   uint64_t hist_bytes;
   uint64_t partition_bytes;
   uint32_t pass_kernel_launches[2];
+  uint32_t early_pack_files, early_pack_deferred;
+  int32_t  probe_file;
+  uint32_t reserved_;
 } mgc_profile;
 int mgc_set_profiling(mgc_session *s, int enable);
 int mgc_get_profile(const mgc_session *s, mgc_profile *p);
diff --git a/meryl_amd/build.py b/meryl_amd/build.py
--- a/meryl_amd/build.py
+++ b/meryl_amd/build.py
@@ -9,7 +9,7 @@
 SOURCES = ["mgc_kmer.hip", "mgc_sort.hip", "mgc_scan.hip", "mgc_finish.hip", "mgc_misc.hip", "mgc_parse.hip",
            "mgc_encode.hip", "mgc_decode.hip", "mgc_merge.hip", "mgc_merge_many.hip", "mgc_lookup.hip", "mgc_filter.hip", "mgc_import.hip", "mgc_analyze.hip", "mgc_value_hist.hip", "mgc_positions.hip", "mgc_list.hip", "mgc_bam.hip", "mgc_gzip.hip",
            "mgc_api.cpp", "mgc_textfile.cpp", "mgc_import.cpp", "mgc_analyze.cpp", "mgc_dbfile.cpp", "mgc_positions.cpp", "mgc_count.cpp", "mgc_stream.cpp", "mgc_eval.cpp", "mgc_runs.cpp", "mgc_node.cpp", "meryl_db.cpp", "meryl_seq.cpp"]
-HEADERS = ["mgc_device.h", "mgc_common.hpp", "mgc_compact.hpp", "mgc_bases.hpp", "mgc_stream_geom.hpp", "mdb_layout.h", "mdb_statistics.hpp", "mgc_session.hpp", "mgc_devbuf.hpp", "mgc_dbfile.hpp", "mgc_hist_list.hpp", "mgc_clock.hpp", "mgc_chunk_ring.hpp", "mgc_bgzf.hpp", "mgc_bam_walk.hpp", "mgc_gzip_par.hpp", "mgc_runs.hpp", "mgc_lookup_dev.hpp", "mgc_import_dev.hpp", "mgc_analyze_dev.hpp", "mgc_positions_dev.hpp", "mgc_fastx.hpp", "mgc_label.hpp", "mgc_selector.hpp", "mgc_value.hpp", "mgc_route.hpp", "mgc_group_route.hpp", "mgc_group_batch.hpp", "mgc_list.hpp",
+HEADERS = ["mgc_device.h", "mgc_common.hpp", "mgc_compact.hpp", "mgc_bases.hpp", "mgc_stream_geom.hpp", "mdb_layout.h", "mdb_statistics.hpp", "mgc_session.hpp", "mgc_devbuf.hpp", "mgc_dbfile.hpp", "mgc_hist_list.hpp", "mgc_clock.hpp", "mgc_chunk_ring.hpp", "mgc_bgzf.hpp", "mgc_bam_walk.hpp", "mgc_gzip_par.hpp", "mgc_runs.hpp", "mgc_lookup_dev.hpp", "mgc_import_dev.hpp", "mgc_analyze_dev.hpp", "mgc_positions_dev.hpp", "mgc_fastx.hpp", "mgc_label.hpp", "mgc_selector.hpp", "mgc_value.hpp", "mgc_route.hpp", "mgc_group_route.hpp", "mgc_group_batch.hpp", "mgc_pack_plan.hpp", "mgc_list.hpp",
            os.path.join("..", "..", "include", "meryl_gpu_count.h"),
            os.path.join("..", "..", "include", "meryl_db.h"), os.path.join("..", "..", "include", "meryl_seq.h"),
            os.path.join("..", "..", "include", "meryl_lookup.h"), os.path.join("..", "..", "include", "meryl_import.h"),
diff --git a/meryl_amd/capi.py b/meryl_amd/capi.py
--- a/meryl_amd/capi.py
+++ b/meryl_amd/capi.py
@@ -184,6 +184,10 @@
         ("hist_bytes", ctypes.c_uint64),
         ("partition_bytes", ctypes.c_uint64),
         ("pass_kernel_launches", ctypes.c_uint32 * 2),
+        ("early_pack_files", ctypes.c_uint32),
+        ("early_pack_deferred", ctypes.c_uint32),
+        ("probe_file", ctypes.c_int32),
+        ("reserved_", ctypes.c_uint32),
     ]
 
 
diff --git a/meryl_amd/csrc/mgc_api.cpp b/meryl_amd/csrc/mgc_api.cpp
--- a/meryl_amd/csrc/mgc_api.cpp
+++ b/meryl_amd/csrc/mgc_api.cpp
@@ -41,6 +41,9 @@
   sw.pass_stagger = (uint32_t)num("MGC_PASS_STAGGER", 0);
   sw.group_batch_bytes = num("MGC_GROUP_BATCH_BYTES", sw.group_batch_bytes);
   sw.group_batch_files = (uint32_t)num("MGC_GROUP_BATCH_FILES", 0);
+  sw.pack_overlap = !off("MGC_PACK_OVERLAP");
+  { const char *e = getenv("MGC_PACK_MARGIN"); if (e && *e) sw.pack_margin = strtoll(e, nullptr, 10); }
+  sw.pack_ratio = (uint32_t)num("MGC_PACK_RATIO", 0);
   return sw;
 }
 }
@@ -676,6 +679,8 @@
   if (s->h_stats) (void)hipHostFree(s->h_stats);
   if (s->ev_join) (void)hipEventDestroy(s->ev_join);
   if (s->stream2) (void)hipStreamDestroy(s->stream2);
+  for (hipEvent_t e : s->pack_ev) (void)hipEventDestroy(e);
+  if (s->ev_pack_done) (void)hipEventDestroy(s->ev_pack_done);
   for (int i = 0; i < mgc_session::HUGE_EXTRA; i++) if (s->stream_h[i]) (void)hipStreamDestroy(s->stream_h[i]);
   if (s->stream) (void)hipStreamDestroy(s->stream);
   delete s;
diff --git a/meryl_amd/csrc/mgc_count.cpp b/meryl_amd/csrc/mgc_count.cpp
--- a/meryl_amd/csrc/mgc_count.cpp
+++ b/meryl_amd/csrc/mgc_count.cpp
@@ -1,6 +1,7 @@
 #include "mgc_session.hpp"
 #include "mgc_group_batch.hpp"
 #include "mgc_group_route.hpp"
+#include "mgc_pack_plan.hpp"
 
 #include <algorithm>
 #include <vector>
@@ -287,6 +288,14 @@
   int n_huge_streams = 1, huge_next = 0;
   std::vector<std::pair<hipEvent_t, hipEvent_t>> fin_ev;
   uint64_t fin_keys = 0, fin_in_bytes = 0; bool fin_narrow = false;
+  bool early = false;
+  std::vector<uint32_t> chain;
+  std::vector<int> chain_pos;
+  std::vector<char> pack_ev2;
+  uint64_t *d_pstate = nullptr;
+  hipStream_t pack_st = nullptr;
+  uint64_t early_cap = 0;
+  hipEvent_t ev_pack[2] = {nullptr, nullptr};
 
   Count(mgc_session *s_, const mgc::CountInput &in_, uint32_t bucket_bits_)
       : s(s_), in(in_), st(s_->stream), c(s_->cfg), sw(s_->sw), prof(s_->prof), k(c.k), kw(s_->key_words), bucket_bits(bucket_bits_),
@@ -314,7 +323,9 @@
   int huge_setup(); int huge_sync_all(); int huge_join_all();
   int finish_file(uint32_t b); int oversized_streams(uint32_t b, bool *stream); int widen_back(uint32_t b, bool *unordered);
   int count_file(uint32_t b, bool stream); int fallback_file(uint32_t b, bool unordered);
-  int trace_slices(); int retry(); int scan_pack(); int pack_file(uint32_t b); void finish_profile();
+  int trace_slices(); int retry(); int scan_pack(); void finish_profile();
+  int pack_file(uint32_t b, hipStream_t ps, const uint64_t *d_gate = nullptr, uint64_t gate_above = 0);
+  int pack_events(); int pack_plan(); int pack_step(uint32_t b); int pack_finish(); int pack_done();
   int block_offsets(); void collect_profile();
 };
 
@@ -829,6 +840,11 @@
   }
   HIP_TRY(s, mgc::launch_finish_file(finish_desc(b, stream, fst, hsel)));
   if (s->profiling) (void)hipEventRecord(fin_ev.back().second, fst);
+  if ((size_t)nb + b < s->pack_ev.size()) {
+    HIP_TRY(s, hipEventRecord(s->pack_ev[b], fst));
+    pack_ev2[b] = stream && x.nlarge > 0 && hstream[hsel] != fst;
+    if (pack_ev2[b]) HIP_TRY(s, hipEventRecord(s->pack_ev[(size_t)nb + b], hstream[hsel]));
+  }
   return MGC_OK;
 }
 
@@ -880,7 +896,6 @@
 }
 
 int Count::scan_pack() {
-  hipEvent_t ev_pack[2] = {nullptr, nullptr};
   if (s->profiling) { (void)hipEventCreate(&ev_pack[0]); (void)hipEventCreate(&ev_pack[1]); (void)hipEventRecord(ev_pack[0], st); }
   HIP_TRY(s, mgc::launch_finish_scan(d_group, plan.ng_total, s->buf[S::B_GSCAN].p, st));
   HIP_TRY(s, hipMemcpyAsync(&nd, d_group + plan.ng_total, sizeof(uint64_t), hipMemcpyDeviceToHost, st));
@@ -896,7 +911,11 @@
     s->d_unique = s->buf[S::B_UNIQUE].p;
     s->d_counts = reinterpret_cast<uint32_t *>(s->buf[S::B_COUNTS].p);
   }
-  for (uint32_t b = 0; b < nb; b++) TRY(pack_file(b));
+  for (uint32_t b = 0; b < nb; b++) TRY(pack_file(b, st));
+  return pack_done();
+}
+
+int Count::pack_done() {
   if (s->profiling) (void)hipEventRecord(ev_pack[1], st);
   tm.end(MGC_STAGE_RLE);
   prof.stage_launches[MGC_STAGE_RLE] = 4 * nb;
@@ -909,25 +928,144 @@
   return MGC_OK;
 }
 
-int Count::pack_file(uint32_t b) {
+int Count::pack_file(uint32_t b, hipStream_t ps, const uint64_t *d_gate, uint64_t gate_above) {
   const FilePlan &x = plan.files[b];
   if (x.size == 0) return MGC_OK;
   void *sg = seg(b);
   if (x.kind == Group::NARROW) {
     HIP_TRY(s, mgc::launch_compact_groups_narrow(sg, x.cnt, d_substart + x.sbase, d_group + x.gbase, x.ngf(), (uint64_t)b << rem_bits, low(x),
-                                                 s->d_unique, s->d_counts, st, x.tr_a, x.tr_b, nz_list(x), x.nzcount));
+                                                 s->d_unique, s->d_counts, ps, x.tr_a, x.tr_b, nz_list(x), x.nzcount, d_gate, gate_above));
   } else if (!x.fallback && x.k96) {
     const unsigned __int128 fb = (unsigned __int128)b << rem_bits;
     HIP_TRY(s, mgc::launch_compact_groups_k96(sg, x.cnt, d_substart + x.sbase, d_group + x.gbase, x.ngf(), (uint64_t)fb, (uint64_t)(fb >> 64),
-                                              s->d_unique, s->d_counts, st, x.tr_a, x.tr_b, nz_list(x), x.nzcount));
+                                              s->d_unique, s->d_counts, ps, x.tr_a, x.tr_b, nz_list(x), x.nzcount, d_gate, gate_above));
   } else if (!x.fallback) {
-    HIP_TRY(s, mgc::launch_compact_groups(sg, kw, x.cnt, d_substart + x.sbase, d_group + x.gbase, x.ngf(), s->d_unique, s->d_counts, st,
-                                          x.tr_a, x.tr_b, nz_list(x), x.nzcount));
+    HIP_TRY(s, mgc::launch_compact_groups(sg, kw, x.cnt, d_substart + x.sbase, d_group + x.gbase, x.ngf(), s->d_unique, s->d_counts, ps,
+                                          x.tr_a, x.tr_b, nz_list(x), x.nzcount, d_gate, gate_above));
   } else {
-    HIP_TRY(s, mgc::launch_rle_count(sg, x.size, kw, rle_ws, st));
-    HIP_TRY(s, mgc::launch_rle_emit(sg, x.size, kw, rle_ws, s->d_unique, s->d_counts, st, d_group + x.gbase));
-  }
-  return MGC_OK;
+    HIP_TRY(s, mgc::launch_rle_count(sg, x.size, kw, rle_ws, ps));
+    HIP_TRY(s, mgc::launch_rle_emit(sg, x.size, kw, rle_ws, s->d_unique, s->d_counts, ps, d_group + x.gbase));
+  }
+  return MGC_OK;
+}
+
+int Count::pack_events() {
+  if (!sw.pack_overlap) return MGC_OK;
+  pack_ev2.assign(nb, 0);
+  while (s->pack_ev.size() < 2 * (size_t)nb) {
+    hipEvent_t e = nullptr;
+    HIP_TRY(s, hipEventCreateWithFlags(&e, hipEventDisableTiming));
+    s->pack_ev.push_back(e);
+  }
+  return MGC_OK;
+}
+
+int Count::pack_plan() {
+  if (!sw.pack_overlap || s->pack_ev.size() < 2 * (size_t)nb) return MGC_OK;
+  std::vector<mgc::PackFile> pf(nb);
+  uint32_t listed = 0;
+  for (uint32_t b = 0; b < nb; b++) {
+    const FilePlan &x = plan.files[b];
+    pf[b] = mgc::PackFile{x.size, x.maxsub, x.nlarge, mgc::finish_uses_hash(kw, low(x)), x.fallback};
+    listed += x.size && x.nlarge ? 1u : 0u;
+  }
+  const bool eligible = mgc::pack_overlap_eligible(pf, plan.cap, sw.stream_max, true);
+  if (sw.finish_trace) fprintf(stderr, "[finish] early packing: %u files have an oversized list; the count is %s\n", listed, eligible ? "eligible" : "not eligible");
+  if (!eligible) return MGC_OK;
+  if (s->worker_active || !s->st_in || n_huge_streams > 1) return MGC_OK;
+  pack_st = s->st_in;
+  const bool caller = in.out_keys && in.out_counts;
+  auto arena_kmers = [&]() { return mgc::pack_buffers_kmers(s->buf[S::B_UNIQUE].cap, s->buf[S::B_COUNTS].cap, kbytes); };
+  const double ratio = probe >= 0 ? prof.probe_ratio : (double)sw.pack_ratio / 1000.0;
+  const uint64_t est = mgc::pack_estimate(ratio, N, sw.pack_margin);
+  const uint64_t want = mgc::pack_arena_want(caller, est, arena_kmers());
+  if (want && (s->ensure(S::B_UNIQUE, kbytes * want) != hipSuccess || s->ensure(S::B_COUNTS, sizeof(uint32_t) * want) != hipSuccess))
+    (void)hipGetLastError();
+  early_cap = mgc::pack_capacity(caller, in.out_cap, arena_kmers());
+  if (sw.finish_trace) fprintf(stderr, "[finish] early packing: %llu k-mers, %llu distinct expected (%s %.4f, margin %lld/1000), room for %llu%s\n",
+                               (unsigned long long)N, (unsigned long long)est, probe >= 0 ? "probe file's ratio" : (sw.pack_ratio ? "MGC_PACK_RATIO" : "no probe file: ratio"), ratio, (long long)sw.pack_margin,
+                               (unsigned long long)early_cap, caller ? " in the caller's buffers" : "");
+  if (early_cap == 0) return MGC_OK;
+  if (!s->ev_pack_done && hipEventCreateWithFlags(&s->ev_pack_done, hipEventDisableTiming) != hipSuccess) { s->ev_pack_done = nullptr; (void)hipGetLastError(); return MGC_OK; }
+  chain_pos.assign(nb, -1);
+  for (uint32_t b = 0; b < nb; b++) if (plan.files[b].size) { chain_pos[b] = (int)chain.size(); chain.push_back(b); }
+  uint64_t max_slice = 0;
+  for (size_t i = 0; i < chain.size(); i++)
+    max_slice = std::max(max_slice, (i + 1 < chain.size() ? plan.files[chain[i + 1]].gbase : plan.ng_total) - plan.files[chain[i]].gbase);
+  HIP_TRY(s, s->ensure(S::B_PACK_STATE, mgc::pack_state_bytes((uint32_t)chain.size(), max_slice)));
+  d_pstate = reinterpret_cast<uint64_t *>(s->buf[S::B_PACK_STATE].p);
+  s->d_unique = caller ? in.out_keys : s->buf[S::B_UNIQUE].p;
+  s->d_counts = caller ? in.out_counts : reinterpret_cast<uint32_t *>(s->buf[S::B_COUNTS].p);
+  HIP_TRY(s, mgc::launch_pack_state_init(d_pstate, early_cap, pack_st));
+  early = true;
+  return MGC_OK;
+}
+
+int Count::pack_step(uint32_t b) {
+  if (!early || chain_pos[b] < 0) return MGC_OK;
+  const FilePlan &x = plan.files[b];
+  const uint64_t i = (uint64_t)chain_pos[b], m = chain.size();
+  hipStream_t ps = pack_st;
+  HIP_TRY(s, hipStreamWaitEvent(ps, s->pack_ev[b], 0));
+  if (pack_ev2[b]) HIP_TRY(s, hipStreamWaitEvent(ps, s->pack_ev[(size_t)nb + b], 0));
+  const uint64_t g1 = i + 1 < m ? plan.files[chain[i + 1]].gbase : plan.ng_total;
+  HIP_TRY(s, mgc::launch_pack_gate_scan(d_group + x.gbase, g1 - x.gbase, d_pstate, (uint32_t)m, (uint32_t)i, x.stream ? d_retrycnt + b : nullptr,
+                                        i + 1 == m ? d_group + plan.ng_total : nullptr, false, ps));
+  if (i > 0) TRY(pack_file(chain[i - 1], ps, d_pstate, mgc::pack_gate_threshold(i - 1, m)));
+  if (i + 1 == m) TRY(pack_file(b, ps, d_pstate, mgc::pack_gate_threshold(i, m)));
+  return MGC_OK;
+}
+
+int Count::pack_finish() {
+  const uint64_t m = chain.size(), none = mgc::pack_state_none();
+  if (s->profiling) { (void)hipEventCreate(&ev_pack[0]); (void)hipEventCreate(&ev_pack[1]); (void)hipEventRecord(ev_pack[0], st); }
+  HIP_TRY(s, hipEventRecord(s->ev_pack_done, pack_st));
+  HIP_TRY(s, hipStreamWaitEvent(st, s->ev_pack_done, 0));
+  std::vector<uint64_t> h(3 + m + 1, 0);
+  HIP_TRY(s, hipMemcpyAsync(h.data(), d_pstate, sizeof(uint64_t) * h.size(), hipMemcpyDeviceToHost, st));
+  HIP_TRY(s, hipStreamSynchronize(st));
+  const uint64_t q = h[0] == none ? m : std::min<uint64_t>(h[0], m);
+  for (uint64_t i = 0; i < m; i++) prof.early_pack_files += mgc::pack_ran_early(i, q, m) ? 1u : 0u;
+  prof.early_pack_deferred = (uint32_t)(m - q);
+  if (sw.finish_trace) {
+    double lo = 2.0, hi = 0.0;
+    for (uint64_t i = 0; i < q; i++) { const double r = (double)(h[3 + i + 1] - h[3 + i]) / (double)plan.files[chain[i]].size; lo = std::min(lo, r); hi = std::max(hi, r); }
+    fprintf(stderr, "[finish] early packing: %llu of %llu files scanned before the last count kernel ended (%u packed), %llu distinct in them, "
+                    "distinct / instances per file %.4f .. %.4f\n", (unsigned long long)q, (unsigned long long)m, prof.early_pack_files,
+            (unsigned long long)h[3 + q], q ? lo : 0.0, hi);
+  }
+  if (q == m) {
+    nd = h[3 + m];
+    s->n_distinct = nd;
+    return pack_done();
+  }
+  TRY(retry());
+  if (s->profiling) (void)hipEventRecord(ev_pack[0], st);
+  for (uint64_t i = q; i < m; i++) {
+    const FilePlan &x = plan.files[chain[i]];
+    const uint64_t g1 = i + 1 < m ? plan.files[chain[i + 1]].gbase : plan.ng_total;
+    HIP_TRY(s, mgc::launch_pack_gate_scan(d_group + x.gbase, g1 - x.gbase, d_pstate, (uint32_t)m, (uint32_t)i, nullptr,
+                                          i + 1 == m ? d_group + plan.ng_total : nullptr, true, st));
+  }
+  HIP_TRY(s, hipMemcpyAsync(&nd, d_group + plan.ng_total, sizeof(uint64_t), hipMemcpyDeviceToHost, st));
+  HIP_TRY(s, hipStreamSynchronize(st));
+  s->n_distinct = nd;
+  const void *was_keys = s->d_unique; const uint32_t *was_counts = s->d_counts;
+  bool moved = false;
+  if (in.out_keys && in.out_counts && nd <= in.out_cap) {
+    s->d_unique = in.out_keys;
+    s->d_counts = in.out_counts;
+  } else {
+    moved = s->buf[S::B_UNIQUE].cap < std::max<size_t>(kbytes * nd, 256) || s->buf[S::B_COUNTS].cap < std::max<size_t>(sizeof(uint32_t) * nd, 256);
+    HIP_TRY(s, s->ensure(S::B_UNIQUE, kbytes * nd));
+    HIP_TRY(s, s->ensure(S::B_COUNTS, sizeof(uint32_t) * nd));
+    s->d_unique = s->buf[S::B_UNIQUE].p;
+    s->d_counts = reinterpret_cast<uint32_t *>(s->buf[S::B_COUNTS].p);
+  }
+  moved = moved || s->d_unique != was_keys || s->d_counts != was_counts;
+  if (moved) prof.early_pack_files = 0;
+  for (uint64_t i = moved ? 0 : mgc::pack_late_from(q, m); i < m; i++) TRY(pack_file(chain[i], st));
+  return pack_done();
 }
 
 void Count::finish_profile() {
@@ -969,11 +1107,18 @@
   hstream[0] = fork_huge ? s->stream2 : st;
   halt[0] = Y;
   hws_bytes = mgc::finish_huge_workspace_bytes(plan.max_bucket);
+  TRY(pack_events());
+  prof.probe_file = probe;
   if (probe >= 0) TRY(probe_file());
   TRY(group_all());
-  for (uint32_t b = 0; b < nb; b++) if ((int)b != probe) TRY(finish_file(b));
+  TRY(pack_plan());
+  for (uint32_t b = 0; b < nb; b++) {
+    if ((int)b != probe) TRY(finish_file(b));
+    TRY(pack_step(b));
+  }
   if (need_join) TRY(huge_join_all());
   TRY(trace_slices());
+  if (early) return pack_finish();
   TRY(retry());
   return scan_pack();
 }
@@ -1043,6 +1188,7 @@
   HIP_TRY(s, hipSetDevice(s->device));
   const uint32_t bucket_bits = in.keys ? in.bucket_bits : plan_bucket_bits(s->cfg, s->sw, s->n_bases);
   memset(&s->prof, 0, sizeof(s->prof));
+  s->prof.probe_file = -1;
   Count count(s, in, bucket_bits);
   return count.run();
 }
diff --git a/meryl_amd/csrc/mgc_device.h b/meryl_amd/csrc/mgc_device.h
--- a/meryl_amd/csrc/mgc_device.h
+++ b/meryl_amd/csrc/mgc_device.h
@@ -35,6 +35,9 @@
   uint64_t bucket_bases = 0;
   uint64_t group_batch_bytes = (uint64_t)1 << 40;
   uint32_t group_batch_files = 0;
+  bool     pack_overlap = true;
+  int64_t  pack_margin = 64;
+  uint32_t pack_ratio = 0;
 };
 Switches read_switches();
 
@@ -199,13 +202,21 @@
 hipError_t launch_compact_groups(const void *d_keys, uint32_t key_words, const uint32_t *d_cnt_tmp, const uint64_t *d_starts,
                                  const uint64_t *d_offs, uint64_t ng, void *d_out_keys, uint32_t *d_out_counts, hipStream_t st,
                                  uint32_t tr_a = 0, uint32_t tr_b = 0 ,
-                                 const uint32_t *d_nonempty_list = nullptr, uint64_t n_nonempty = 0 );
+                                 const uint32_t *d_nonempty_list = nullptr, uint64_t n_nonempty = 0 ,
+                                 const uint64_t *d_gate = nullptr, uint64_t gate_above = 0 );
 hipError_t launch_compact_groups_narrow(const void *d_keys32, const uint32_t *d_cnt_tmp, const uint64_t *d_starts, const uint64_t *d_offs,
                                         uint64_t ng, uint64_t base, uint32_t low_bits, void *d_out_keys, uint32_t *d_out_counts, hipStream_t st,
-                                        uint32_t tr_a, uint32_t tr_b, const uint32_t *d_nonempty_list = nullptr, uint64_t n_nonempty = 0);
+                                        uint32_t tr_a, uint32_t tr_b, const uint32_t *d_nonempty_list = nullptr, uint64_t n_nonempty = 0,
+                                        const uint64_t *d_gate = nullptr, uint64_t gate_above = 0);
 hipError_t launch_compact_groups_k96(const void *d_keys96, const uint32_t *d_cnt_tmp, const uint64_t *d_starts, const uint64_t *d_offs,
                                      uint64_t ng, uint64_t base_lo, uint64_t base_hi, void *d_out_keys, uint32_t *d_out_counts, hipStream_t st,
-                                     uint32_t tr_a, uint32_t tr_b, const uint32_t *d_nonempty_list = nullptr, uint64_t n_nonempty = 0);
+                                     uint32_t tr_a, uint32_t tr_b, const uint32_t *d_nonempty_list = nullptr, uint64_t n_nonempty = 0,
+                                     const uint64_t *d_gate = nullptr, uint64_t gate_above = 0);
+size_t     pack_state_bytes(uint32_t n_files, uint64_t max_slice);
+uint64_t   pack_state_none();
+hipError_t launch_pack_state_init(uint64_t *d_state, uint64_t capacity, hipStream_t st);
+hipError_t launch_pack_gate_scan(uint64_t *d_slice, uint64_t n, uint64_t *d_state, uint32_t n_files, uint32_t i, const uint64_t *d_retry_count,
+                                 uint64_t *d_total, bool force, hipStream_t st);
 hipError_t launch_widen_k96(const void *d_keys96, uint64_t n, uint64_t base_lo, uint64_t base_hi, void *d_out128, hipStream_t st);
 hipError_t launch_widen_groups(const void *d_keys32, const uint64_t *d_starts, uint64_t ng, uint64_t base, uint32_t low_bits, void *d_out64,
                                hipStream_t st, uint32_t tr_a, uint32_t tr_b);
diff --git a/meryl_amd/csrc/mgc_finish.hip b/meryl_amd/csrc/mgc_finish.hip
--- a/meryl_amd/csrc/mgc_finish.hip
+++ b/meryl_amd/csrc/mgc_finish.hip
@@ -2089,7 +2089,9 @@
 __global__ __launch_bounds__(256)
 void compact_groups_kernel(const K *__restrict__ keys, const u32 *__restrict__ cnt_tmp, const u64 *__restrict__ starts,
                            const u64 *__restrict__ offs, u64 ng, K *__restrict__ out_keys, u32 *__restrict__ out_counts, u32 tr_a, u32 tr_b,
-                           const u32 *__restrict__ nz, u64 n_nz ) {
+                           const u32 *__restrict__ nz, u64 n_nz ,
+                           const u64 *__restrict__ gate, u64 gate_above ) {
+  if (gate && *gate <= gate_above) return;
   u64 g = (u64)blockIdx.x * 4 + wave_id();
   if (nz) { if (g >= n_nz) return; g = nz[g]; }
   else if (g >= ng) return;
@@ -2104,7 +2106,9 @@
 __global__ __launch_bounds__(256)
 void compact_groups_k96_kernel(const K96 *__restrict__ keys, const u32 *__restrict__ cnt_tmp, const u64 *__restrict__ starts,
                                const u64 *__restrict__ offs, u64 ng, u64 base_lo, u64 base_hi, K128 *__restrict__ out_keys,
-                               u32 *__restrict__ out_counts, u32 tr_a, u32 tr_b, const u32 *__restrict__ nz, u64 n_nz) {
+                               u32 *__restrict__ out_counts, u32 tr_a, u32 tr_b, const u32 *__restrict__ nz, u64 n_nz,
+                               const u64 *__restrict__ gate, u64 gate_above) {
+  if (gate && *gate <= gate_above) return;
   u64 g = (u64)blockIdx.x * 4 + wave_id();
   if (nz) { if (g >= n_nz) return; g = nz[g]; }
   else if (g >= ng) return;
@@ -2129,7 +2133,9 @@
 __global__ __launch_bounds__(256)
 void compact_groups_narrow_kernel(const u32 *__restrict__ keys32, const u32 *__restrict__ cnt_tmp, const u64 *__restrict__ starts,
                                   const u64 *__restrict__ offs, u64 ng, u64 base, u32 low_bits, u64 *__restrict__ out_keys,
-                                  u32 *__restrict__ out_counts, u32 tr_a, u32 tr_b, const u32 *__restrict__ nz, u64 n_nz) {
+                                  u32 *__restrict__ out_counts, u32 tr_a, u32 tr_b, const u32 *__restrict__ nz, u64 n_nz,
+                               const u64 *__restrict__ gate, u64 gate_above) {
+  if (gate && *gate <= gate_above) return;
   u64 g = (u64)blockIdx.x * 4 + wave_id();
   if (nz) { if (g >= n_nz) return; g = nz[g]; }
   else if (g >= ng) return;
@@ -2574,39 +2580,119 @@
                             reinterpret_cast<u64 *>(d_group) + ng_total, st);
 }
 
+constexpr u64 PACK_NONE = ~0ull;
+constexpr int PG_BLOCK = 256, PG_ITEMS = 16, PG_CHUNK = PG_BLOCK * PG_ITEMS;
+__global__ __launch_bounds__(PG_BLOCK)
+void pack_chunk_sums_kernel(const u64 *__restrict__ grp, u64 n, u64 *__restrict__ chunk_tot) {
+  __shared__ u64 s_tmp[PG_BLOCK / 64 + 1];
+  const u64 c0 = (u64)blockIdx.x * PG_CHUNK;
+  u64 v = 0;
+#pragma unroll
+  for (int q = 0; q < PG_ITEMS; q++) {
+    const u64 j = c0 + (u64)q * PG_BLOCK + threadIdx.x;
+    v += j < n ? grp[j] : 0ull;
+  }
+  u64 tot;
+  (void)block_excl_scan<PG_BLOCK, u64>(v, s_tmp, &tot);
+  if (threadIdx.x == 0) chunk_tot[blockIdx.x] = tot;
+}
+
+__global__ __launch_bounds__(PG_BLOCK)
+void pack_gate_scan_kernel(u64 *__restrict__ grp, u64 n, u64 *state, u32 i, const u64 *__restrict__ retry_count,
+                           u64 *__restrict__ total_out, u32 force, const u64 *__restrict__ chunk_tot) {
+  __shared__ u64 s_tmp[PG_BLOCK / 64 + 1];
+  __shared__ u32 s_go;
+  const u32 tid = threadIdx.x, c = blockIdx.x, nchunks = gridDim.x;
+  if (!force) {
+    if (tid == 0) s_go = (state[0] == PACK_NONE) ? ((retry_count && *retry_count != 0) ? 1u : 2u) : 0u;
+    __syncthreads();
+    if (s_go == 0) return;
+  }
+  u64 pre = 0, all = 0;
+  for (u32 j = tid; j < nchunks; j += PG_BLOCK) { const u64 t = chunk_tot[j]; all += t; pre += j < c ? t : 0ull; }
+  u64 pre_tot, all_tot;
+  (void)block_excl_scan<PG_BLOCK, u64>(pre, s_tmp, &pre_tot);
+  (void)block_excl_scan<PG_BLOCK, u64>(all, s_tmp, &all_tot);
+  const u64 base = state[3 + i];
+  if (!force && (s_go == 1 || base + all_tot > state[1])) { if (c == 0 && tid == 0) state[0] = i; return; }
+  const u64 c0 = (u64)c * PG_CHUNK;
+  u64 v[PG_ITEMS], sum = 0;
+#pragma unroll
+  for (int q = 0; q < PG_ITEMS; q++) {
+    const u64 j = c0 + (u64)tid * PG_ITEMS + q;
+    v[q] = j < n ? grp[j] : 0ull;
+    sum += v[q];
+  }
+  u64 tot;
+  u64 run = base + pre_tot + block_excl_scan<PG_BLOCK, u64>(sum, s_tmp, &tot);
+#pragma unroll
+  for (int q = 0; q < PG_ITEMS; q++) {
+    const u64 j = c0 + (u64)tid * PG_ITEMS + q;
+    if (j < n) grp[j] = run;
+    run += v[q];
+  }
+  if (c + 1 == nchunks && tid == 0) {
+    state[3 + i + 1] = base + all_tot;
+    if (total_out) *total_out = base + all_tot;
+  }
+}
+
+__global__ void pack_state_init_kernel(u64 *__restrict__ state, u64 capacity) {
+  state[0] = PACK_NONE; state[1] = capacity; state[2] = 0; state[3] = 0;
+}
+
+static uint64_t pack_chunks(uint64_t n) { return (n + PG_CHUNK - 1) / PG_CHUNK; }
+size_t pack_state_bytes(uint32_t n_files, uint64_t max_slice) { return sizeof(uint64_t) * (3 + (size_t)n_files + 1 + (size_t)pack_chunks(max_slice)); }
+uint64_t pack_state_none() { return PACK_NONE; }
+hipError_t launch_pack_state_init(uint64_t *d_state, uint64_t capacity, hipStream_t st) {
+  hipLaunchKernelGGL(pack_state_init_kernel, dim3(1), dim3(1), 0, st, reinterpret_cast<u64 *>(d_state), (u64)capacity);
+  return hipGetLastError();
+}
+hipError_t launch_pack_gate_scan(uint64_t *d_slice, uint64_t n, uint64_t *d_state, uint32_t n_files, uint32_t i, const uint64_t *d_retry_count,
+                                 uint64_t *d_total, bool force, hipStream_t st) {
+  if (n == 0 || i >= n_files) return hipErrorInvalidValue;
+  u64 *chunk_tot = reinterpret_cast<u64 *>(d_state) + 3 + (size_t)n_files + 1;
+  const dim3 grid((uint32_t)pack_chunks(n));
+  hipLaunchKernelGGL(pack_chunk_sums_kernel, grid, dim3(PG_BLOCK), 0, st, reinterpret_cast<const u64 *>(d_slice), (u64)n, chunk_tot);
+  MGC_CHECK(hipGetLastError());
+  hipLaunchKernelGGL(pack_gate_scan_kernel, grid, dim3(PG_BLOCK), 0, st, reinterpret_cast<u64 *>(d_slice), (u64)n, reinterpret_cast<u64 *>(d_state), i,
+                     reinterpret_cast<const u64 *>(d_retry_count), reinterpret_cast<u64 *>(d_total), force ? 1u : 0u, (const u64 *)chunk_tot);
+  return hipGetLastError();
+}
+
 hipError_t launch_compact_groups(const void *d_keys, uint32_t key_words, const uint32_t *d_cnt_tmp, const uint64_t *d_starts,
                                  const uint64_t *d_offs, uint64_t ng, void *d_out_keys, uint32_t *d_out_counts, hipStream_t st,
-                                 uint32_t tr_a, uint32_t tr_b, const uint32_t *d_nz, uint64_t n_nz) {
+                                 uint32_t tr_a, uint32_t tr_b, const uint32_t *d_nz, uint64_t n_nz, const uint64_t *d_gate, uint64_t gate_above) {
   const dim3 grid((uint32_t)(((d_nz ? n_nz : ng) + 3) / 4));
   if (d_nz && n_nz == 0) return hipSuccess;
   if (key_words == 2)
     hipLaunchKernelGGL(compact_groups_kernel<K128>, grid, dim3(256), 0, st, reinterpret_cast<const K128 *>(d_keys), d_cnt_tmp,
                        reinterpret_cast<const u64 *>(d_starts), reinterpret_cast<const u64 *>(d_offs), (u64)ng,
-                       reinterpret_cast<K128 *>(d_out_keys), d_out_counts, tr_a, tr_b, d_nz, (u64)n_nz);
+                       reinterpret_cast<K128 *>(d_out_keys), d_out_counts, tr_a, tr_b, d_nz, (u64)n_nz, reinterpret_cast<const u64 *>(d_gate), (u64)gate_above);
   else
     hipLaunchKernelGGL(compact_groups_kernel<u64>, grid, dim3(256), 0, st, reinterpret_cast<const u64 *>(d_keys), d_cnt_tmp,
                        reinterpret_cast<const u64 *>(d_starts), reinterpret_cast<const u64 *>(d_offs), (u64)ng,
-                       reinterpret_cast<u64 *>(d_out_keys), d_out_counts, tr_a, tr_b, d_nz, (u64)n_nz);
+                       reinterpret_cast<u64 *>(d_out_keys), d_out_counts, tr_a, tr_b, d_nz, (u64)n_nz, reinterpret_cast<const u64 *>(d_gate), (u64)gate_above);
   return hipGetLastError();
 }
 
 hipError_t launch_compact_groups_narrow(const void *d_keys32, const uint32_t *d_cnt_tmp, const uint64_t *d_starts, const uint64_t *d_offs,
                                         uint64_t ng, uint64_t base, uint32_t low_bits, void *d_out_keys, uint32_t *d_out_counts, hipStream_t st,
-                                        uint32_t tr_a, uint32_t tr_b, const uint32_t *d_nz, uint64_t n_nz) {
+                                        uint32_t tr_a, uint32_t tr_b, const uint32_t *d_nz, uint64_t n_nz, const uint64_t *d_gate, uint64_t gate_above) {
   if (d_nz && n_nz == 0) return hipSuccess;
   hipLaunchKernelGGL(compact_groups_narrow_kernel, dim3((uint32_t)(((d_nz ? n_nz : ng) + 3) / 4)), dim3(256), 0, st, reinterpret_cast<const u32 *>(d_keys32),
                      d_cnt_tmp, reinterpret_cast<const u64 *>(d_starts), reinterpret_cast<const u64 *>(d_offs), (u64)ng, (u64)base, low_bits,
-                     reinterpret_cast<u64 *>(d_out_keys), d_out_counts, tr_a, tr_b, d_nz, (u64)n_nz);
+                     reinterpret_cast<u64 *>(d_out_keys), d_out_counts, tr_a, tr_b, d_nz, (u64)n_nz, reinterpret_cast<const u64 *>(d_gate), (u64)gate_above);
   return hipGetLastError();
 }
 
 hipError_t launch_compact_groups_k96(const void *d_keys96, const uint32_t *d_cnt_tmp, const uint64_t *d_starts, const uint64_t *d_offs,
                                      uint64_t ng, uint64_t base_lo, uint64_t base_hi, void *d_out_keys, uint32_t *d_out_counts, hipStream_t st,
-                                     uint32_t tr_a, uint32_t tr_b, const uint32_t *d_nz, uint64_t n_nz) {
+                                     uint32_t tr_a, uint32_t tr_b, const uint32_t *d_nz, uint64_t n_nz, const uint64_t *d_gate, uint64_t gate_above) {
   if (d_nz && n_nz == 0) return hipSuccess;
   hipLaunchKernelGGL(compact_groups_k96_kernel, dim3((uint32_t)(((d_nz ? n_nz : ng) + 3) / 4)), dim3(256), 0, st, reinterpret_cast<const K96 *>(d_keys96),
                      d_cnt_tmp, reinterpret_cast<const u64 *>(d_starts), reinterpret_cast<const u64 *>(d_offs), (u64)ng, (u64)base_lo, (u64)base_hi,
-                     reinterpret_cast<K128 *>(d_out_keys), d_out_counts, tr_a, tr_b, d_nz, (u64)n_nz);
+                     reinterpret_cast<K128 *>(d_out_keys), d_out_counts, tr_a, tr_b, d_nz, (u64)n_nz, reinterpret_cast<const u64 *>(d_gate), (u64)gate_above);
   return hipGetLastError();
 }
 
diff --git a/meryl_amd/csrc/mgc_pack_plan.hpp b/meryl_amd/csrc/mgc_pack_plan.hpp
--- /dev/null
+++ b/meryl_amd/csrc/mgc_pack_plan.hpp
@@ -0,0 +1,53 @@
+#pragma once
+#include <cstddef>
+#include <cstdint>
+#include <vector>
+
+namespace mgc {
+
+struct PackFile { uint64_t size, maxsub, nlarge; bool hash, fallback; };
+
+inline bool pack_file_ok(const PackFile &f, uint64_t cap, uint64_t stream_max) {
+  if (f.size == 0) return true;
+  if (f.fallback) return false;
+  return f.nlarge == 0 ? f.maxsub <= cap : (f.hash && f.maxsub <= stream_max);
+}
+
+inline bool pack_overlap_eligible(const std::vector<PackFile> &files, uint64_t cap, uint64_t stream_max, bool switch_on) {
+  bool any = false;
+  for (const PackFile &f : files) {
+    if (!pack_file_ok(f, cap, stream_max)) return false;
+    any = any || f.size != 0;
+  }
+  return switch_on && any;
+}
+
+constexpr int64_t PACK_MARGIN_PERMILLE = 64;
+constexpr uint64_t PACK_MARGIN_FLOOR = 4096;
+
+inline uint64_t pack_estimate(double probe_ratio, uint64_t instances, int64_t margin_permille) {
+  if (!(probe_ratio > 0.0) || instances == 0) return 0;
+  const double r = probe_ratio < 1.0 ? probe_ratio : 1.0;
+  double e = r * (double)instances * (1.0 + (double)margin_permille / 1000.0);
+  if (e < 0.0) e = 0.0;
+  const uint64_t est = (e >= (double)instances ? instances : (uint64_t)e) + (margin_permille >= 0 ? PACK_MARGIN_FLOOR : 0);
+  return est < instances ? est : instances;
+}
+
+inline uint64_t pack_arena_want(bool caller_buffers, uint64_t estimate, uint64_t arena_kmers) {
+  if (caller_buffers || estimate <= arena_kmers) return 0;
+  return estimate;
+}
+
+inline uint64_t pack_capacity(bool caller_buffers, uint64_t out_cap, uint64_t arena_kmers) { return caller_buffers ? out_cap : arena_kmers; }
+
+inline uint64_t pack_buffers_kmers(size_t key_buf_bytes, size_t count_buf_bytes, size_t key_bytes) {
+  const uint64_t a = key_buf_bytes / key_bytes, b = count_buf_bytes / sizeof(uint32_t);
+  return a < b ? a : b;
+}
+
+inline bool pack_ran_early(uint64_t i, uint64_t q, uint64_t m) { return i + 1 < q || (i + 1 == m && q == m); }
+inline uint64_t pack_late_from(uint64_t q, uint64_t m) { return q >= m ? m : (q ? q - 1 : 0); }
+inline uint64_t pack_gate_threshold(uint64_t i, uint64_t m) { return i + 1 < m ? i + 1 : i; }
+
+}
diff --git a/meryl_amd/csrc/mgc_session.hpp b/meryl_amd/csrc/mgc_session.hpp
--- a/meryl_amd/csrc/mgc_session.hpp
+++ b/meryl_amd/csrc/mgc_session.hpp
@@ -53,6 +53,8 @@
   hipStream_t      stream_h[HUGE_EXTRA] = {nullptr, nullptr, nullptr};
   hipStream_t      stream2 = nullptr;
   hipEvent_t       ev_fork = nullptr, ev_join = nullptr;
+  std::vector<hipEvent_t> pack_ev;
+  hipEvent_t       ev_pack_done = nullptr;
   uint64_t        *h_stats = nullptr;
   size_t           h_stats_cap = 0;
   std::string      err;
@@ -76,7 +78,8 @@
          B_PACKED ,
          B_GROUP_BATCH ,
          B_BAM_SEG0, B_BAM_SEG1 ,
-         B_GZ_SYM0, B_GZ_SYM1 , B_GZ_TAB0, B_GZ_TAB1 , B_GZ_WIN , B_NUM };
+         B_GZ_SYM0, B_GZ_SYM1 , B_GZ_TAB0, B_GZ_TAB1 , B_GZ_WIN ,
+         B_PACK_STATE , B_NUM };
   Buf buf[B_NUM];
   size_t arena_bytes() const { size_t t = 0; for (const auto &b : buf) t += b.cap; return t; }
   double tr_alloc = 0;
```

Measured after the change: 12.84 billion distinct k-mers/s (median of 6 runs). 1.03x the previous value.
